# pghysels/STRUMPACK

Hardware: AMD Instinct MI355X
Metric: hss_compress_ulv_factor_solve_gflops (higher is better)
Workload: dtype f64

## Files before the change

### include/hssk.h

```cpp
#ifndef HSSK_H
#define HSSK_H

#ifdef __cplusplus
extern "C" {
#endif

typedef struct hssk_ctx hssk_ctx;

int hssk_ctx_create(hssk_ctx** ctx, int device);
void hssk_ctx_destroy(hssk_ctx* ctx);
void* hssk_ctx_stream(hssk_ctx* ctx);
int hssk_sync(hssk_ctx* ctx);
const char* hssk_last_error(void);
typedef struct hssk_plan hssk_plan;
int hssk_plan_begin(hssk_ctx* ctx, hssk_plan** plan);
int hssk_plan_end(hssk_ctx* ctx);
int hssk_plan_replay(hssk_ctx* ctx, hssk_plan* plan);
void hssk_plan_destroy(hssk_plan* plan);
int hssk_plan_size(const hssk_plan* plan);

void* hssk_malloc(long long bytes);
void hssk_free(void* dptr);
long long hssk_device_total_bytes(void);
int hssk_memcpy_h2d(hssk_ctx* ctx, void* dst, const void* src, long long bytes);
int hssk_memcpy_d2h(hssk_ctx* ctx, void* dst, const void* src, long long bytes);
int hssk_upload_async(hssk_ctx* ctx, void* dst, const void* src, long long bytes);
int hssk_memcpy_d2d(hssk_ctx* ctx, void* dst, const void* src, long long bytes);
int hssk_memcpy2d_h2d(hssk_ctx* ctx, void* dst, long long dpitch, const void* src, long long spitch,
                      long long width, long long height);
int hssk_memcpy2d_d2h(hssk_ctx* ctx, void* dst, long long dpitch, const void* src, long long spitch,
                      long long width, long long height);
int hssk_memset_zero(hssk_ctx* ctx, void* dst, long long bytes);
int hssk_h2d_block_async(hssk_ctx* ctx, double* dst, long long ldd, const double* src, long long lds, long long rows,
                         long long cols);
int hssk_h2d_bytes_async(hssk_ctx* ctx, void* dst, long long dpitch, const void* src, long long spitch, long long width,
                         long long cols);
int hssk_copy_fence(hssk_ctx* ctx);
int hssk_compute_fence(hssk_ctx* ctx);
int hssk_compute_mark(hssk_ctx* ctx, int slot);
int hssk_copy_wait(hssk_ctx* ctx, int slot);
int hssk_is_device_pointer(const void* ptr);
typedef struct hssk_aca_desc {
  const double* A;
  int lda, m, n;
  double rtol, atol;
  int max_rank, row0;
  double* U;
  int ldu;
  double* V;
  int ldv;
  int* rank;
} hssk_aca_desc;
int hssk_aca_vbatched(hssk_ctx* ctx, const hssk_aca_desc* descs, int count);
int hssk_side_begin(hssk_ctx* ctx);
int hssk_side_end(hssk_ctx* ctx);
int hssk_side_join(hssk_ctx* ctx);
int hssk_stream_wait(hssk_ctx* waiter, hssk_ctx* on);
int hssk_watch_start(hssk_ctx* ctx, int id);
int hssk_watch_stop(hssk_ctx* ctx, int id);
double hssk_watch_read_ms(hssk_ctx* ctx, int id, int* pairs);
float hssk_last_dgemm_ms(hssk_ctx* ctx);
double hssk_last_dgemm_flops(hssk_ctx* ctx);
int hssk_dgemm_timing_defer(hssk_ctx* ctx);
int hssk_dgemm_timing_collect(hssk_ctx* ctx, double* ms, double* flops, int* launches);
long long hssk_last_dgemm_trace(hssk_ctx* ctx, long long* out, long long max_wgs);
double hssk_last_dgemm_clock_ghz(hssk_ctx* ctx);

int hssk_fill_toeplitz(hssk_ctx* ctx, double* A, int n, long long lda, char kind);
int hssk_fill_toeplitz_block(hssk_ctx* ctx, double* A, int rows, int cols, long long lda, int i0, int j0, char kind);
int hssk_randn(hssk_ctx* ctx, double* P, int rows, long long cols, long long ld, int row0,
               long long stride, unsigned long long seed);

int hssk_dgemm(hssk_ctx* ctx, int transB, int m, long long n, long long k, double alpha,
               const double* A, long long lda, const double* B, long long ldb, double beta,
               double* C, long long ldc);

int hssk_sgemm_sketch(hssk_ctx* ctx, int transB, int m, long long n, long long k, double alpha,
                      const double* A, long long lda,
                      const float* B, long long ldb,
                      double beta, double* C, long long ldc);
int hssk_narrow_f32(hssk_ctx* ctx, float* dst, long long ldd, const double* src, long long lds, long long rows, long long cols);

#define HSSK_GEN_TOEPLITZ 1
#define HSSK_GEN_TOEPLITZ_UPPER 2
typedef struct hssk_gen {
  int kind, reserved;
  double p[4];
} hssk_gen;
int hssk_sketch_gen(hssk_ctx* ctx, const hssk_gen* g, int transG, int m, long long n, long long k, long long j0, double alpha,
                    const double* A, long long lda, double beta, double* C, long long ldc);
int hssk_gen_fill(hssk_ctx* ctx, const hssk_gen* g, double* A, long long rows, long long cols, long long lda, long long i0,
                  long long j0, int trans);

typedef struct hssk_gemm_desc {
  const double* A;
  const double* B;
  double* C;
  int m, n, k;
  int lda, ldb, ldc;
  int transA, transB;
  double alpha, beta;
} hssk_gemm_desc;
int hssk_gemm_vbatched(hssk_ctx* ctx, const hssk_gemm_desc* descs, int count);

typedef struct hssk_leaf_update_desc {
  const double* R;
  const double* D;
  double* Sr;
  double* Sc;
  int d, m, ldr, ldd, lds;
} hssk_leaf_update_desc;
int hssk_leaf_update_vbatched(hssk_ctx* ctx, const hssk_leaf_update_desc* descs, int count);

typedef struct hssk_kernel_spec {
  const double* X;
  long long n;
  int d, type, p;
  double h, lambda;
} hssk_kernel_spec;
typedef struct hssk_keval_desc {
  const int* ri;
  const int* ci;
  double* out;
  int nr, nc, ldo, r0, c0;
} hssk_keval_desc;
int hssk_kernel_eval_vbatched(hssk_ctx* ctx, const hssk_kernel_spec* spec, const hssk_keval_desc* descs, int count);
int hssk_knn(hssk_ctx* ctx, const double* X, int d, int n, int k, int q0, int q1, int* out_idx);
typedef struct hssk_colset_desc {
  const int* src0;
  const int* src1;
  int n0, n1, lo, hi;
  int* out;
  int* count;
  const int* n0_dev;
  const int* n1_dev;
} hssk_colset_desc;
int hssk_colsets(hssk_ctx* ctx, const hssk_colset_desc* descs, int count, int universe);
long long hssk_colsets_max_universe(void);
int hssk_cluster_median(hssk_ctx* ctx, double* X, int d, int n, int algo, int cluster_size, int* perm, int* status);
int hssk_kernel_predict(hssk_ctx* ctx, const hssk_kernel_spec* spec, const double* w, const double* T, int m, double* pred);
#define HSSK_KPREDICT_TAU 1.220703125e-4
int hssk_kernel_predict_f32(hssk_ctx* ctx, const float* X, long long n, int d, int type, int p, double h,
                            const float* w, const float* T, int m, float* pred, long long* stats);
int hssk_kernel_predict_splits(long long n, int m);

typedef struct hssk_colgather_desc {
  const double* src;
  double* dst;
  const int* idx;
  int rows, ncols, lds, ldd;
  int scatter;
} hssk_colgather_desc;
int hssk_gather_cols(hssk_ctx* ctx, const hssk_colgather_desc* descs, int count);
enum { HSSK_DT_F64 = 0, HSSK_DT_F32 = 1, HSSK_DT_C32 = 2, HSSK_DT_C64 = 3 };
int hssk_expand_image(hssk_ctx* ctx, double* dst, long long ldd, const void* src, long long lds, long long rows, long long cols,
                      int dtype);
typedef struct hssk_rowgather_desc {
  const double* src;
  double* dst;
  const int* idx;
  int nrows, cols, lds, ldd;
  int scatter, accumulate;
} hssk_rowgather_desc;
int hssk_gather_rows(hssk_ctx* ctx, const hssk_rowgather_desc* descs, int count);
typedef struct hssk_elem_desc {
  const double* A;
  long long lda;
  const int* I;
  const int* J;
  int i0, j0;
  double* B;
  int m, n, ldb, transpose;
  int rlo, rhi, clo, chi;
} hssk_elem_desc;
int hssk_gather_elems(hssk_ctx* ctx, const hssk_elem_desc* descs, int count);
int hssk_gather_elems_f32(hssk_ctx* ctx, const hssk_elem_desc* descs, int count);
int hssk_gen_elems(hssk_ctx* ctx, const hssk_gen* g, const hssk_elem_desc* descs, int count);
int hssk_sum_slabs(hssk_ctx* ctx, const double* slabs, long long count, long long stride, int nslab, double* out);
typedef struct hssk_transpose_desc {
  const double* src;
  double* dst;
  int rows, cols, lds, ldd;
} hssk_transpose_desc;
int hssk_transpose(hssk_ctx* ctx, const hssk_transpose_desc* descs, int count);

typedef struct hssk_triu_desc {
  const double* src;
  double* dst;
  int rows, cols, lds, ldd;
  int dstride;
} hssk_triu_desc;
int hssk_copy_triu(hssk_ctx* ctx, const hssk_triu_desc* descs, int count);

int hssk_sjlt_dense(hssk_ctx* ctx, double* Rt, int dn, long long K, long long ld, const int* pat, int nnz);
int hssk_sjlt_sketch(hssk_ctx* ctx, int transA, long long n_out, long long K, const double* A, long long lda,
                     const int* pat, int nnz, int dn, double* St, long long lds);

typedef struct hssk_combine_desc {
  const double *G0, *G1;
  int ldg, gsplit;
  const int* gidx;
  const double *M0, *M1;
  int ldm, msplit;
  const int* midx;
  const double* C;
  int csj, csk;
  double alpha;
  double* out;
  int ldo, rows, J, K;
} hssk_combine_desc;
int hssk_gather_combine(hssk_ctx* ctx, const hssk_combine_desc* descs, int count);

typedef struct hssk_ulvsplit_desc {
  const double* D;
  int ldd, m, r;
  const int* perm;
  const double* X;
  int ldx;
  double* W1;
  int ldw;
  double* W0t;
  int ldt;
} hssk_ulvsplit_desc;
int hssk_ulv_split(hssk_ctx* ctx, const hssk_ulvsplit_desc* descs, int count);
typedef struct hssk_ulvnode_desc {
  const double *B01, *B10, *Vt1a, *Vt1b, *Vd;
  double *Dh, *Vh;
  int ra, rb, rva, rvb;
  int eliminate;
  const int* perm;
  const double* X;
  double *W1, *Rlq, *Qt, *tau, *Vt0T, *Vt1, *Dt, *WQ;
  int m, r, rv, ldt;
} hssk_ulvnode_desc;
int hssk_ulv_node_vbatched(hssk_ctx* ctx, const hssk_ulvnode_desc* descs, int count);
int hssk_ulv_node_fits(int m, int r, int rv, int ra, int rb, int rva, int rvb);
long long hssk_ulv_node_launches(void);

typedef struct hssk_id_desc {
  double* W;
  int ldw, d, m;
  double rtol, atol;
  int max_rank;
  int* perm;
  int* rank;
  double* work;
  const double* src;
  int lds;
  int defer_x;
} hssk_id_desc;
int hssk_id_vbatched(hssk_ctx* ctx, const hssk_id_desc* descs, int count);
long long hssk_id_group_launches(void);
int hssk_id_solves_inline(int dmax, int mmax);
typedef struct hssk_xsolve_desc {
  const double* W;
  int ldw, rank, m;
  double* X;
  int ldx, solved;
} hssk_xsolve_desc;
int hssk_id_xsolve_vbatched(hssk_ctx* ctx, const hssk_xsolve_desc* descs, int count);
typedef struct hssk_pchol_desc {
  const double* G;
  int ldg, m;
  double rtol, atol;
  int max_rank;
  int* perm;
  int* rank;
  double* R;
  int ldr;
} hssk_pchol_desc;
int hssk_pchol_id_vbatched(hssk_ctx* ctx, const hssk_pchol_desc* descs, int count);
int hssk_pchol_id_max_m(void);
int hssk_pchol_id_rank_cap(int m);
typedef struct hssk_sum_desc {
  const double* P;
  long long stride, n;
  int count;
  double* out;
} hssk_sum_desc;
int hssk_sum_partials(hssk_ctx* ctx, const hssk_sum_desc* descs, int count);
typedef struct hssk_gram_desc {
  const double* W;
  int ldw, rows, m;
  double* G;
  int ldg;
} hssk_gram_desc;
int hssk_gram_vbatched(hssk_ctx* ctx, const hssk_gram_desc* descs, int count);
typedef struct hssk_gramgen_desc {
  const int* ri;
  int r0;
  const int* ci;
  int c0;
  int rows, m;
  double* G;
  int ldg;
} hssk_gramgen_desc;
int hssk_gram_gen_vbatched(hssk_ctx* ctx, const hssk_kernel_spec* spec, const hssk_gramgen_desc* descs, int count);
int hssk_gram_gen_supported(const hssk_kernel_spec* spec, int mmax);

typedef struct hssk_tnode {
  int c0, c1, lvl, reserved;
  double* S[2];
  int* perm[2];
  double* Rred[2];
  int* I[2];
  double* X[2];
  double *B01, *B10;
  double* W[2];
  int r[2], m[2], flag[2];
  int status, pad;
} hssk_tnode;
typedef struct hssk_elem_src {
  const double* A;
  long long lda;
  hssk_gen gen;
  int use_gen;
} hssk_elem_src;
int hssk_tree_inner(hssk_ctx* ctx, hssk_tnode* nodes, const int* order, int count, int d, int lds, int rcap, double rtol,
                    double atol, int max_rank, const hssk_elem_src* src, int* res);
int hssk_tree_rcap_max(void);

typedef struct hssk_qr_desc {
  double* A;
  int lda, rows, cols;
  double* Q;
  int ldq, nq;
  double* rdiag;
  double* work;
  int stair;
  double stop_rel, stop_abs;
  int r_only;
} hssk_qr_desc;
int hssk_qr_vbatched(hssk_ctx* ctx, const hssk_qr_desc* descs, int count);
typedef struct hssk_tpqr_desc {
  double* R1;
  int ld1;
  const double* R2;
  int ld2, m;
} hssk_tpqr_desc;
int hssk_tpqr_vbatched(hssk_ctx* ctx, const hssk_tpqr_desc* descs, int count);
int hssk_formq_vbatched(hssk_ctx* ctx, const hssk_qr_desc* descs, int count);

typedef struct hssk_trsm_desc {
  const double* T;
  double* B;
  int n, nrhs, ldt, ldb;
  int lower, transT, unit;
  const double* Tinv;
} hssk_trsm_desc;
int hssk_trsm_vbatched(hssk_ctx* ctx, const hssk_trsm_desc* descs, int count);
typedef struct hssk_lu_desc {
  double* A;
  int n, lda;
  int* piv;
  int* info;
} hssk_lu_desc;
int hssk_getrf_vbatched(hssk_ctx* ctx, const hssk_lu_desc* descs, int count);
typedef struct hssk_lusolve_desc {
  const double* LU;
  const int* piv;
  double* B;
  int n, nrhs, lda, ldb;
} hssk_lusolve_desc;
int hssk_getrs_vbatched(hssk_ctx* ctx, const hssk_lusolve_desc* descs, int count);
int hssk_laswp_vbatched(hssk_ctx* ctx, const hssk_lusolve_desc* descs, int count);

typedef struct hssk_blr_term {
  const double* U;
  const double* V;
  int r, n, src_off, src_flag;
} hssk_blr_term;
typedef struct hssk_blr_row {
  int first_term, nterms, off, m;
  const double* LU;
  int lda, mode;
  const int* piv;
  const double* Tinv;
} hssk_blr_row;
int hssk_blr_sweep(hssk_ctx* ctx, const hssk_blr_row* rows, int nrows, const hssk_blr_term* terms, int nterms, double* X, int* flags);
int hssk_blr_sweep_check(const hssk_blr_row* rows, int nrows, const hssk_blr_term* terms, int nterms);
int hssk_blr_sweep_resident(hssk_ctx* ctx, const hssk_blr_row* d_rows, int nrows, const hssk_blr_term* d_terms, double* X, int* flags);

int hssk_sweep_arm(hssk_ctx* ctx, double* handoff, long long count);
typedef struct hssk_sweep_fwd_desc {
  const double* fsrc;
  const double *B01, *B10, *zc;
  const int* permU;
  const double* XU;
  const double* Rlq;
  const double* Tinv;
  const double* WQ;
  const double* Vt0T;
  const int* permV;
  const double* XV;
  double *ft1, *y, *z;
  const double *LU, *TinvL, *TinvU;
  const int* piv;
  double* xroot;
  int ldf, rU0, rU1, rV0, rV1, ldz_in, m, r, mv, rv, ldp, ldz, ldxr;
  int wait0, wait1;
  const double* G;
  int ldg;
} hssk_sweep_fwd_desc;
int hssk_sweep_chain_ok(int m, int r, int mv, int rv);
long long hssk_sweep_chain_launches(void);
int hssk_ulv_fwd_sweep(hssk_ctx* ctx, const hssk_sweep_fwd_desc* descs, int count, int nrhs);
typedef struct hssk_sweep_bwd_desc {
  const double *Qt, *y, *xpart;
  double* out;
  int m, r, ldx, ldo;
  int wait0;
} hssk_sweep_bwd_desc;
int hssk_ulv_bwd_sweep(hssk_ctx* ctx, const hssk_sweep_bwd_desc* descs, int count, int nrhs);
typedef struct hssk_apply_up_desc {
  const double* src;
  const int* perm;
  const double* X;
  double* dst;
  int m, r, lds, ldd;
  int inner;
  int wait0, wait1;
} hssk_apply_up_desc;
typedef struct hssk_apply_down_desc {
  const double* tmp2;
  const int* perm;
  const double* X;
  const double *D, *x;
  const double *B01, *B10, *t1;
  double* out;
  double beta;
  int ld2, mo, ro, m, ldx, trans, ri_a, ri_b, ro_a, ro_b, ldt1, ldo;
  int wait0, wait1, wait2;
  int acc;
} hssk_apply_down_desc;
int hssk_apply_sweep(hssk_ctx* ctx, const hssk_apply_up_desc* ups, int nup, const hssk_apply_down_desc* downs, int ndown,
                     int nrhs);
int hssk_sweep_status(hssk_ctx* ctx);
int hssk_sweep_require_mma(hssk_ctx* ctx, int on);
int hssk_sweep_mma_min_nrhs(void);
long long hssk_sweep_mma_launches(void);
long long hssk_sweep_fused_launches(void);
long long hssk_sweep_fallbacks(void);
typedef struct hssk_trtri_desc {
  const double* R;
  double* Tinv;
  int n, ldr;
  int mode;
} hssk_trtri_desc;
int hssk_trtri_diag_vbatched(hssk_ctx* ctx, const hssk_trtri_desc* descs, int count);

typedef struct hssk_tree_node {
  int lo, m, c0, c1;
  int rU, rV, mU, mV;
  const double *XU, *XV;
  const int *ipermU, *ipermV;
  const double *B01, *B10, *D;
} hssk_tree_node;
typedef struct hssk_extract_block {
  int ri0, ni, cj0, nj;
  double* out;
  int ldo;
} hssk_extract_block;
int hssk_hss_extract(hssk_ctx* ctx, const hssk_tree_node* nodes, int root, int rmax, int maxdepth, const int* rows, int nrows,
                     const int* cols, int ncols, const hssk_extract_block* blocks, const long long* pair_off, int nblocks,
                     long long npairs, int accumulate, double* work);

typedef struct hssk_norm_desc {
  const double* P;
  int rows, cols, ld;
  double* out;
} hssk_norm_desc;
int hssk_sumsq_vbatched(hssk_ctx* ctx, const hssk_norm_desc* descs, int count);
typedef struct hssk_basis_desc {
  const double* X;
  const int* perm;
  double* out;
  int m, r, ldx, ldo;
} hssk_basis_desc;
int hssk_basis_dense(hssk_ctx* ctx, const hssk_basis_desc* descs, int count);
typedef struct hssk_shift_desc {
  double* A;
  int n, lda;
} hssk_shift_desc;
int hssk_shift_diag(hssk_ctx* ctx, const hssk_shift_desc* descs, int count, double sigma);
int hssk_shift_diag_cplx(hssk_ctx* ctx, const hssk_shift_desc* descs, int count, double re, double im);
double hssk_mfma_f64_peak_tflops(hssk_ctx* ctx, int iters);
int hssk_mfma_f64_probe(hssk_ctx* ctx, int iters, int waves_per_simd, int zero_data, double* out);

#ifdef __cplusplus
}
#endif
#endif
```

### strumpack_amd/csrc/host/hss_sources.cpp

```cpp
#include "hss_engine_internal.hpp"

namespace strumpack {
namespace HSS {

double DeviceHSS::Source::sketch_flops(const DeviceHSS& H, int dn) const {
  return 2.0 * products(H) * (double)H.n_ * (double)H.n_ * (H.sj_pat_ ? H.sj_nnz_ : dn);
}

struct DeviceHSS::DenseDeviceSource : DeviceHSS::Source {
  const double* dA;
  long long lda;
  DenseDeviceSource(const double* a, long long l) : dA(a), lda(l) {}
  bool extract_before_sample() const override { return true; }
  bool device_elems(const DeviceHSS&, hssk_elem_src* e) const override { e->A = dA; e->lda = lda; e->use_gen = 0; return true; }
  int done_products_ = 2;
  bool done_sparse_ = false;
  int products(const DeviceHSS&) const override { return done_products_; }
  double sketch_flops(const DeviceHSS& H, int dn) const override {
    return 2.0 * done_products_ * (double)H.n_ * (double)H.n_ * (done_sparse_ ? H.sj_nnz_ : dn);
  }
  void sample(DeviceHSS& H, int r0, int dn) override {
    const long long N = H.n_;
    long long j0 = 0, j1 = N;
    if (H.dist_subtree_) {
      const Node& c = H.nodes_[H.cut_nodes_[H.o_.rank]];
      j0 = c.lo; j1 = c.lo + c.m;
    } else if (H.o_.world > 1) {
      j0 = std::min(N, H.cols_per_rank_ * H.o_.rank); j1 = std::min(N, j0 + H.cols_per_rank_);
    }
    const long long nloc = j1 - j0;
    static const bool sj_dense = std::getenv("STRUMPACK_AMD_SJLT_DENSE") && std::atoi(std::getenv("STRUMPACK_AMD_SJLT_DENSE"));
    done_sparse_ = H.sj_pat_ && dn <= 1024 && !sj_dense;
    done_products_ = (!done_sparse_ && H.o_.symmetric) ? 1 : 2;
    if (nloc > 0 && done_sparse_) {
      for (int t = 0; t < 2; t++) {
        const double* Aop = t == 0 ? dA + j0 : dA + j0 * lda;
        double* St = (t == 0 ? H.Srt_ : H.Sct_) + r0 + j0 * H.dcap_;
        ck(hssk_sjlt_sketch(H.ctx_, t, nloc, N, Aop, lda, H.sj_pat_, H.sj_nnz_, dn, St, H.dcap_));
        ck(hssk_sync(H.ctx_));
        float ms = hssk_last_dgemm_ms(H.ctx_);
        if (ms > 0) {
          H.stats_.sketch_kernel_ms += ms; H.stats_.sketch_launches++;
          H.stats_.sketch_kernel_flops += hssk_last_dgemm_flops(H.ctx_);
          H.stats_.sketch_kernel_bytes += 8.0 * (double)nloc * (double)N;
        }
      }
    } else if (nloc > 0) {
      ck(hssk_dgemm(H.ctx_, 1, dn, nloc, N, 1.0, H.Rt_ + r0, H.dcap_, dA + j0, lda, 0.0, H.Srt_ + r0 + j0 * H.dcap_, H.dcap_));
      ck(hssk_dgemm_timing_defer(H.ctx_));
      if (H.o_.symmetric) {
        hssk_colgather_desc cp{H.Srt_ + r0 + j0 * H.dcap_, H.Sct_ + r0 + j0 * H.dcap_, nullptr, dn, (int)nloc, H.dcap_, H.dcap_, 0};
        ck(hssk_gather_cols(H.ctx_, &cp, 1));
      } else {
        ck(hssk_dgemm(H.ctx_, 0, dn, nloc, N, 1.0, H.Rt_ + r0, H.dcap_, dA + j0 * lda, lda, 0.0, H.Sct_ + r0 + j0 * H.dcap_, H.dcap_));
        ck(hssk_dgemm_timing_defer(H.ctx_));
      }
    }
    if (H.o_.world > 1 && !H.dist_subtree_) {
      const long long bytes = (long long)sizeof(double) * H.dcap_ * H.cols_per_rank_;
      H.comm(H.Srt_, bytes);
      H.comm(H.Sct_, bytes);
    }
  }
  void extract(DeviceHSS& H, const std::vector<ElemReq>& reqs) override {
    std::vector<hssk_elem_desc> d;
    d.reserve(reqs.size());
    for (auto& r : reqs)
      if (r.m > 0 && r.n > 0) d.push_back(hssk_elem_desc{dA, lda, r.dI, r.dJ, r.i0, r.j0, r.dB, r.m, r.n, r.ldb, 0});
    if (!d.empty()) ck(hssk_gather_elems(H.ctx_, d.data(), (int)d.size()));
  }
};

struct DeviceHSS::DenseDeviceSourceF32 : DeviceHSS::Source {
  const float* dA;
  long long lda;
  int route;
  double* dBuf = nullptr;
  long long nb = 0;
  int gen = -1;
  int done_products_ = 2;
  DenseDeviceSourceF32(const float* a, long long l, int r) : dA(a), lda(l), route(r) {}
  bool extract_before_sample() const override { return true; }
  bool device_elems(const DeviceHSS&, hssk_elem_src* e) const override {
    e->A = reinterpret_cast<const double*>(dA); e->lda = lda; e->use_gen = 2;
    return true;
  }
  int products(const DeviceHSS&) const override { return done_products_; }
  double sketch_flops(const DeviceHSS& H, int dn) const override { return 2.0 * done_products_ * (double)H.n_ * (double)H.n_ * dn; }
  void sample(DeviceHSS& H, int r0, int dn) override {
    if (H.o_.world > 1) throw std::invalid_argument("single-precision device operand: single-GPU only (multi-GPU float operands are not supported)");
    if (H.sj_pat_) throw std::invalid_argument("single-precision device operand: the SJLT sketch is not supported; use the Gaussian sketch");
    const long long N = H.n_;
    if (N <= 0 || dn <= 0) return;
    auto timed = [&](double bytes) {
      ck(hssk_dgemm_timing_defer(H.ctx_));
      H.stats_.sketch_kernel_bytes += bytes;
    };
    if (route == 1) {
      done_products_ = H.o_.symmetric ? 1 : 2;
      ck(hssk_sgemm_sketch(H.ctx_, 1, dn, N, N, 1.0, H.Rt_ + r0, H.dcap_, dA, lda, 0.0, H.Srt_ + r0, H.dcap_));
      timed(4.0 * (double)N * (double)N);
      if (H.o_.symmetric) {
        hssk_colgather_desc cp{H.Srt_ + r0, H.Sct_ + r0, nullptr, dn, (int)N, H.dcap_, H.dcap_, 0};
        ck(hssk_gather_cols(H.ctx_, &cp, 1));
      } else {
        ck(hssk_sgemm_sketch(H.ctx_, 0, dn, N, N, 1.0, H.Rt_ + r0, H.dcap_, dA, lda, 0.0, H.Sct_ + r0, H.dcap_));
        timed(4.0 * (double)N * (double)N);
      }
      return;
    }
    done_products_ = 2;
    if (gen != H.attempt_) {
      gen = H.attempt_;
      nb = std::max<long long>(64, (1LL << 30) / (8 * N) / 64 * 64);
      nb = std::min(nb, (N + 63) / 64 * 64);
      dBuf = H.work_->dbl((size_t)N * nb);
    }
    for (long long c0 = 0, b = 0; c0 < N; c0 += nb, b++) {
      const long long c1 = std::min(N, c0 + nb);
      ck(hssk_expand_image(H.ctx_, dBuf, N, dA + c0 * lda, lda, N, c1 - c0, HSSK_DT_F32));
      ck(hssk_dgemm(H.ctx_, 0, dn, c1 - c0, N, 1.0, H.Rt_ + r0, H.dcap_, dBuf, N, 0.0, H.Sct_ + r0 + c0 * H.dcap_, H.dcap_));
      timed(0.);
      ck(hssk_dgemm(H.ctx_, 1, dn, N, c1 - c0, 1.0, H.Rt_ + r0 + c0 * H.dcap_, H.dcap_, dBuf, N, b ? 1.0 : 0.0, H.Srt_ + r0, H.dcap_));
      timed(0.);
    }
  }
  void extract(DeviceHSS& H, const std::vector<ElemReq>& reqs) override {
    std::vector<hssk_elem_desc> d;
    d.reserve(reqs.size());
    for (auto& r : reqs)
      if (r.m > 0 && r.n > 0) d.push_back(hssk_elem_desc{reinterpret_cast<const double*>(dA), lda, r.dI, r.dJ, r.i0, r.j0, r.dB, r.m, r.n, r.ldb, 0});
    if (!d.empty()) ck(hssk_gather_elems_f32(H.ctx_, d.data(), (int)d.size()));
  }
};

struct DeviceHSS::ShardedDenseSource : DeviceHSS::Source {
  const double* dRows;
  long long ldr;
  const double* dCols;
  long long ldc;
  ShardedDenseSource(const double* r, long long lr, const double* c, long long lc) : dRows(r), ldr(lr), dCols(c), ldc(lc) {}
  bool device_elems(const DeviceHSS& H, hssk_elem_src* e) const override {
    const Node& c = H.nodes_[H.o_.world == 1 ? 0 : H.cut_nodes_[H.o_.rank]];
    e->A = dCols - (long long)c.lo * ldc; e->lda = ldc; e->use_gen = 0;
    return true;
  }
  void sample(DeviceHSS& H, int r0, int dn) override {
    const bool single = H.o_.world == 1;
    if (!single && !H.dist_subtree_) throw std::invalid_argument("sharded operand: the tree cannot be cut into one subtree per rank (world must be a power of two and the tree complete down to that depth)");
    if (H.sj_pat_) throw std::invalid_argument("sharded operand: the SJLT sketch needs the replicated-operand interface");
    const long long N = H.n_;
    const Node& c = H.nodes_[single ? 0 : H.cut_nodes_[H.o_.rank]];
    const long long j0 = c.lo, nloc = c.m;
    auto timed = [&] { ck(hssk_dgemm_timing_defer(H.ctx_)); };
    ck(hssk_dgemm(H.ctx_, 0, dn, nloc, N, 1.0, H.Rt_ + r0, H.dcap_, dCols, ldc, 0.0, H.Sct_ + r0 + j0 * H.dcap_, H.dcap_));
    timed();
    if (dRows) {
      ck(hssk_dgemm(H.ctx_, 1, dn, nloc, N, 1.0, H.Rt_ + r0, H.dcap_, dRows, ldr, 0.0, H.Srt_ + r0 + j0 * H.dcap_, H.dcap_));
      timed();
    } else {
      H.tmp_->rewind();
      double* P = H.tmp_->dbl((size_t)dn * N);
      double* mineP = H.tmp_->dbl((size_t)dn * nloc);
      ck(hssk_dgemm(H.ctx_, 1, dn, N, nloc, 1.0, H.Rt_ + r0 + j0 * H.dcap_, H.dcap_, dCols, ldc, 0.0, P, dn));
      timed();
      const double tc = now();
      std::vector<long long> offs(H.o_.world), counts(H.o_.world);
      for (int g = 0; g < H.o_.world; g++) {
        const Node& cg = H.nodes_[single ? 0 : H.cut_nodes_[g]];
        offs[g] = (long long)cg.lo * dn; counts[g] = (long long)cg.m * dn;
      }
      H.reduce_scatter_sum(P, offs, counts, mineP);
      hssk_colgather_desc cp{mineP, H.Srt_ + r0 + j0 * H.dcap_, nullptr, dn, (int)nloc, dn, H.dcap_, 0};
      ck(hssk_gather_cols(H.ctx_, &cp, 1));
      ck(hssk_sync(H.ctx_));
      H.stats_.t_comm += now() - tc;
    }
  }
  void extract(DeviceHSS& H, const std::vector<ElemReq>& reqs) override {
    const Node& c = H.nodes_[H.o_.world == 1 ? 0 : H.cut_nodes_[H.o_.rank]];
    const int j0 = c.lo, j1 = c.lo + c.m;
    auto inside = [&](const std::vector<int>* h, int i0, int cnt) {
      if (!h) return i0 >= j0 && i0 + cnt <= j1;
      for (int i = 0; i < cnt; i++) if ((*h)[i] < j0 || (*h)[i] >= j1) return false;
      return true;
    };
    std::vector<hssk_elem_desc> own, part, back;
    size_t tot = 0;
    for (auto& r : reqs) if (r.m > 0 && r.n > 0 && !(inside(r.hI, r.i0, r.m) && inside(r.hJ, r.j0, r.n))) tot += (size_t)r.m * r.n;
    double* stage = tot ? H.comm_arena_->dbl(tot) : nullptr;
    size_t off = 0;
    for (auto& r : reqs) {
      if (r.m <= 0 || r.n <= 0) continue;
      if (inside(r.hI, r.i0, r.m) && inside(r.hJ, r.j0, r.n)) {
        own.push_back(hssk_elem_desc{dCols - (long long)j0 * ldc, ldc, r.dI, r.dJ, r.i0, r.j0, r.dB, r.m, r.n, r.ldb, 0, 0, 0, 0, 0});
      } else {
        double* T = stage + off;
        off += (size_t)r.m * r.n;
        if (dRows) part.push_back(hssk_elem_desc{dRows - j0, ldr, r.dI, r.dJ, r.i0, r.j0, T, r.m, r.n, r.m, 0, j0, j1, 0, 0});
        else part.push_back(hssk_elem_desc{dCols - (long long)j0 * ldc, ldc, r.dI, r.dJ, r.i0, r.j0, T, r.m, r.n, r.m, 0, 0, 0, j0, j1});
        back.push_back(hssk_elem_desc{T, r.m, nullptr, nullptr, 0, 0, r.dB, r.m, r.n, r.ldb, 0, 0, 0, 0, 0});
      }
    }
    if (!own.empty()) ck(hssk_gather_elems(H.ctx_, own.data(), (int)own.size()));
    if (!part.empty()) {
      const double tc = now();
      ck(hssk_gather_elems(H.ctx_, part.data(), (int)part.size()));
      H.allreduce_sum(stage, (long long)tot);
      ck(hssk_gather_elems(H.ctx_, back.data(), (int)back.size()));
      H.stats_.t_comm += now() - tc;
    }
  }
};

struct DeviceHSS::HostBlockSource : DeviceHSS::Source {
  const void* hA;
  long long lda;
  int dtype = HSSK_DT_F64;
  const host_fill_t* fill;
  const host_elem_t* elem;
  double* dBuf[2] = {nullptr, nullptr};
  double* dNat[2] = {nullptr, nullptr};
  long long nb = 0;
  int gen = -1;
  std::vector<double*> dcache;
  HostBlockSource(const void* a, long long l, const host_fill_t* f, const host_elem_t* e, int dt = HSSK_DT_F64)
      : hA(a), lda(l), dtype(dt), fill(f), elem(e) {}
  long long reals() const { return dtype == HSSK_DT_C32 || dtype == HSSK_DT_C64 ? 2 : 1; }
  size_t esize() const { return dtype == HSSK_DT_F32 ? 4 : dtype == HSSK_DT_C64 ? 16 : 8; }
  double image_at(size_t I, size_t J) const {
    switch (dtype) {
      case HSSK_DT_F32: return (double)((const float*)hA)[I + J * (size_t)lda];
      case HSSK_DT_C32: {
        const float* z = (const float*)hA + 2 * (I / 2 + (J / 2) * (size_t)lda);
        return (I & 1) == (J & 1) ? (double)z[0] : ((I & 1) ? (double)z[1] : -(double)z[1]);
      }
      case HSSK_DT_C64: {
        const double* z = (const double*)hA + 2 * (I / 2 + (J / 2) * (size_t)lda);
        return (I & 1) == (J & 1) ? z[0] : ((I & 1) ? z[1] : -z[1]);
      }
      default: return ((const double*)hA)[I + J * (size_t)lda];
    }
  }
  void sample(DeviceHSS& H, int r0, int dn) override {
    if (H.o_.world > 1) throw std::invalid_argument("host-resident operands are single-GPU (use the device / sharded interfaces)");
    const long long N = H.n_;
    const bool typed = hA && dtype != HSSK_DT_F64;
    const long long W = typed ? reals() : 1, ns = N / W;
    if (typed && N % W) throw std::logic_error("image dimension of a complex operand must be even");
    const bool first = gen != H.attempt_;
    if (first) {
      gen = H.attempt_;
      long long bytes = 1536LL << 20;
      if (const char* e = std::getenv("STRUMPACK_AMD_HOST_BLOCK_MB")) bytes = std::max(1LL, std::atoll(e)) << 20;
      if (const char* e = std::getenv("STRUMPACK_AMD_HOST_BLOCK_KB")) bytes = std::max(1LL, std::atoll(e)) << 10;
      nb = std::max<long long>(64, bytes / (8 * std::max<long long>(N, 1)) / 64 * 64);
      nb = std::min(nb, (N + 63) / 64 * 64);
      dBuf[0] = H.work_->dbl((size_t)N * nb);
      if (!typed) dBuf[1] = H.work_->dbl((size_t)N * nb);
      else for (int k = 0; k < 2; k++) dNat[k] = H.work_->dbl(((size_t)ns * (size_t)(nb / W) * esize() + 7) / 8);
    }
    const long long nblk = (N + nb - 1) / nb;
    const bool capture = first;
    if (capture) {
      dcache.assign(H.nodes_.size(), nullptr);
      for (size_t id = 0; id < H.nodes_.size(); id++)
        if (H.nodes_[id].leaf() && H.nodes_[id].m > 0) dcache[id] = H.work_->dbl((size_t)H.nodes_[id].m * H.nodes_[id].m);
    }
    std::vector<double> tmp;
    auto upload = [&](long long b) {
      const long long c0 = b * nb, c1 = std::min(N, c0 + nb);
      if (typed)
        ck(hssk_h2d_bytes_async(H.ctx_, dNat[b & 1], (long long)(ns * esize()), (const char*)hA + (size_t)(c0 / W) * lda * esize(),
                                (long long)(lda * esize()), (long long)(ns * esize()), (c1 - c0) / W));
      else if (hA) ck(hssk_h2d_block_async(H.ctx_, dBuf[b & 1], N, (const double*)hA + (size_t)c0 * lda, lda, N, c1 - c0));
      else {
        tmp.resize((size_t)N * (c1 - c0));
        (*fill)(c0, c1, tmp.data());
        ck(hssk_h2d_block_async(H.ctx_, dBuf[b & 1], N, tmp.data(), N, N, c1 - c0));
      }
    };
    upload(0);
    for (long long b = 0; b < nblk; b++) {
      const long long c0 = b * nb, c1 = std::min(N, c0 + nb);
      ck(hssk_copy_fence(H.ctx_));
      const double* Ab = typed ? dBuf[0] : dBuf[b & 1];
      if (typed) {
        ck(hssk_expand_image(H.ctx_, dBuf[0], N, dNat[b & 1], ns, ns, (c1 - c0) / W, dtype));
        ck(hssk_compute_mark(H.ctx_, (int)(b & 1)));
      }
      ck(hssk_dgemm(H.ctx_, 0, dn, c1 - c0, N, 1.0, H.Rt_ + r0, H.dcap_, Ab, N, 0.0, H.Sct_ + r0 + c0 * H.dcap_, H.dcap_));
      ck(hssk_dgemm(H.ctx_, 1, dn, N, c1 - c0, 1.0, H.Rt_ + r0 + c0 * H.dcap_, H.dcap_, Ab, N, b ? 1.0 : 0.0, H.Srt_ + r0, H.dcap_));
      if (capture) {
        std::vector<hssk_colgather_desc> dg;
        for (size_t id = 0; id < H.nodes_.size(); id++) {
          const Node& nd = H.nodes_[id];
          if (!dcache[id]) continue;
          const long long a = std::max<long long>(nd.lo, c0), e = std::min<long long>(nd.lo + nd.m, c1);
          if (a >= e) continue;
          dg.push_back(hssk_colgather_desc{Ab + nd.lo + (size_t)(a - c0) * N, dcache[id] + (size_t)(a - nd.lo) * nd.m, nullptr, nd.m, (int)(e - a),
                                           (int)N, nd.m, 0});
        }
        if (!dg.empty()) ck(hssk_gather_cols(H.ctx_, dg.data(), (int)dg.size()));
      }
      if (!typed) ck(hssk_compute_mark(H.ctx_, (int)(b & 1)));
      if (b + 1 < nblk) {
        ck(hssk_copy_wait(H.ctx_, (int)((b + 1) & 1)));
        upload(b + 1);
      }
    }
    ck(hssk_sync(H.ctx_));
  }
  void extract(DeviceHSS& H, const std::vector<ElemReq>& reqs) override {
    std::vector<size_t> off(reqs.size() + 1, 0);
    for (size_t k = 0; k < reqs.size(); k++) off[k + 1] = off[k] + (size_t)std::max(reqs[k].m, 0) * std::max(reqs[k].n, 0);
    std::vector<const double*> hit(reqs.size(), nullptr);
    if (!dcache.empty()) {
      std::vector<std::pair<int, size_t>> by_lo;
      for (size_t id = 0; id < H.nodes_.size(); id++) if (dcache[id]) by_lo.push_back({H.nodes_[id].lo, id});
      std::sort(by_lo.begin(), by_lo.end());
      std::vector<hssk_colgather_desc> cp;
      for (size_t k = 0; k < reqs.size(); k++) {
        const ElemReq& r = reqs[k];
        if (r.hI || r.hJ || r.i0 != r.j0 || r.m != r.n || r.m <= 0 || gen != H.attempt_) continue;
        auto it = std::lower_bound(by_lo.begin(), by_lo.end(), std::make_pair(r.i0, size_t(0)));
        if (it == by_lo.end() || it->first != r.i0 || H.nodes_[it->second].m != r.m) continue;
        hit[k] = dcache[it->second];
        cp.push_back(hssk_colgather_desc{hit[k], r.dB, nullptr, r.m, r.n, r.m, r.ldb, 0});
      }
      if (!cp.empty()) ck(hssk_gather_cols(H.ctx_, cp.data(), (int)cp.size()));
    }
    for (size_t k = 0; k < reqs.size(); k++)
      if (hit[k]) off[k + 1] = off[k];
      else off[k + 1] = off[k] + (size_t)std::max(reqs[k].m, 0) * std::max(reqs[k].n, 0);
    std::unique_ptr<double[]> img_store(new double[std::max<size_t>(off.back(), 1)]);
    struct { double* p; double* data() { return p; } } img{img_store.get()};
    host_parallel_for(reqs.size(), [&](size_t k) {
      const ElemReq& r = reqs[k];
      if (r.m <= 0 || r.n <= 0 || hit[k]) return;
      double* B = img.data() + off[k];
      if (hA && dtype != HSSK_DT_F64) {
        for (int j = 0; j < r.n; j++) {
          const size_t J = (size_t)(r.hJ ? (*r.hJ)[j] : r.j0 + j);
          for (int i = 0; i < r.m; i++) B[i + (size_t)j * r.m] = image_at((size_t)(r.hI ? (*r.hI)[i] : r.i0 + i), J);
        }
      } else if (hA) {
        for (int j = 0; j < r.n; j++) {
          const double* col = (const double*)hA + (size_t)(r.hJ ? (*r.hJ)[j] : r.j0 + j) * lda;
          if (r.hI) for (int i = 0; i < r.m; i++) B[i + (size_t)j * r.m] = col[(*r.hI)[i]];
          else std::memcpy(B + (size_t)j * r.m, col + r.i0, sizeof(double) * r.m);
        }
      } else {
        std::vector<int> I(r.m), J(r.n);
        for (int i = 0; i < r.m; i++) I[i] = r.hI ? (*r.hI)[i] : r.i0 + i;
        for (int j = 0; j < r.n; j++) J[j] = r.hJ ? (*r.hJ)[j] : r.j0 + j;
        (*elem)(r.m, I.data(), r.n, J.data(), B, r.m);
      }
    });
    for (size_t k = 0; k < reqs.size(); k++) {
      const ElemReq& r = reqs[k];
      if (r.m <= 0 || r.n <= 0 || hit[k]) continue;
      if (r.ldb == r.m) ck(hssk_upload_async(H.ctx_, r.dB, img.data() + off[k], (long long)(sizeof(double) * (off[k + 1] - off[k]))));
      else ck(hssk_memcpy2d_h2d(H.ctx_, r.dB, sizeof(double) * r.ldb, img.data() + off[k], sizeof(double) * r.m, sizeof(double) * r.m, r.n));
    }
  }
};

struct DeviceHSS::CallbackSource : DeviceHSS::Source {
  const host_mult_t* mult;
  const host_sample_t* usample = nullptr;
  const host_elem_t& elem;
  CallbackSource(const host_mult_t& m, const host_elem_t& e) : mult(&m), elem(e) {}
  CallbackSource(const host_sample_t& s, const host_elem_t& e) : mult(nullptr), usample(&s), elem(e) {}
  void sample(DeviceHSS& H, int r0, int dn) override {
    if (H.o_.world > 1) throw std::invalid_argument("the host-callback interface is single-GPU");
    if (usample) {
      const int N = H.n_;
      if (N == 0 || dn == 0) return;
      std::vector<double> R((size_t)N * dn), Sr((size_t)N * dn), Sc((size_t)N * dn);
      (*usample)(N, dn, R.data(), Sr.data(), Sc.data());
      double* dT = H.tmp_->dbl((size_t)N * dn);
      const double* src[3] = {R.data(), Sr.data(), Sc.data()};
      double* dst[3] = {H.Rt_ + r0, H.Srt_ + r0, H.Sct_ + r0};
      for (int q = 0; q < 3; q++) {
        ck(hssk_memcpy_h2d(H.ctx_, dT, src[q], (long long)(sizeof(double) * (size_t)N * dn)));
        hssk_transpose_desc b{dT, dst[q], N, dn, N, H.dcap_};
        ck(hssk_transpose(H.ctx_, &b, 1));
        ck(hssk_sync(H.ctx_));
      }
      return;
    }
    const int N = H.n_;
    if (N == 0 || dn == 0) return;
    double* dT = H.tmp_->dbl((size_t)N * dn);
    std::vector<double> R((size_t)N * dn), S((size_t)N * dn);
    hssk_transpose_desc t{H.Rt_ + r0, dT, dn, N, H.dcap_, N};
    ck(hssk_transpose(H.ctx_, &t, 1));
    ck(hssk_memcpy_d2h(H.ctx_, R.data(), dT, (long long)(sizeof(double) * R.size())));
    for (int pass = 0; pass < 2; pass++) {
      (*mult)(pass == 0 ? 'N' : 'C', N, dn, R.data(), N, S.data(), N);
      ck(hssk_memcpy_h2d(H.ctx_, dT, S.data(), (long long)(sizeof(double) * S.size())));
      hssk_transpose_desc b{dT, (pass == 0 ? H.Srt_ : H.Sct_) + r0, N, dn, N, H.dcap_};
      ck(hssk_transpose(H.ctx_, &b, 1));
      ck(hssk_sync(H.ctx_));
    }
  }
  void extract(DeviceHSS& H, const std::vector<ElemReq>& reqs) override {
    for (auto& r : reqs) {
      if (r.m <= 0 || r.n <= 0) continue;
      std::vector<int> I(r.m), J(r.n);
      for (int i = 0; i < r.m; i++) I[i] = r.hI ? (*r.hI)[i] : r.i0 + i;
      for (int j = 0; j < r.n; j++) J[j] = r.hJ ? (*r.hJ)[j] : r.j0 + j;
      std::vector<double> B((size_t)r.m * r.n);
      elem(r.m, I.data(), r.n, J.data(), B.data(), r.m);
      ck(hssk_memcpy2d_h2d(H.ctx_, r.dB, sizeof(double) * r.ldb, B.data(), sizeof(double) * r.m, sizeof(double) * r.m, r.n));
    }
  }
};

struct DeviceHSS::GeneratorSource : DeviceHSS::Source {
  hssk_gen g;
  explicit GeneratorSource(const hssk_gen& g_) : g(g_) {}
  bool extract_before_sample() const override { return true; }
  bool device_elems(const DeviceHSS&, hssk_elem_src* e) const override { e->A = nullptr; e->lda = 0; e->gen = g; e->use_gen = 1; return true; }
  int products(const DeviceHSS& H) const override { return H.o_.symmetric ? 1 : 2; }
  void sample(DeviceHSS& H, int r0, int dn) override {
    if (H.sj_pat_) throw std::invalid_argument("generated operand: the SJLT sketch streams a stored matrix; use the Gaussian sketch");
    const long long N = H.n_;
    long long j0 = 0, j1 = N;
    if (H.dist_subtree_) {
      const Node& c = H.nodes_[H.cut_nodes_[H.o_.rank]];
      j0 = c.lo; j1 = c.lo + c.m;
    } else if (H.o_.world > 1) {
      j0 = std::min(N, H.cols_per_rank_ * H.o_.rank); j1 = std::min(N, j0 + H.cols_per_rank_);
    }
    const long long nloc = j1 - j0;
    auto timed = [&] { ck(hssk_dgemm_timing_defer(H.ctx_)); };
    if (nloc > 0) {
      ck(hssk_sketch_gen(H.ctx_, &g, 1, dn, nloc, N, j0, 1.0, H.Rt_ + r0, H.dcap_, 0.0, H.Srt_ + r0 + j0 * H.dcap_, H.dcap_));
      timed();
      if (H.o_.symmetric) {
        hssk_colgather_desc cp{H.Srt_ + r0 + j0 * H.dcap_, H.Sct_ + r0 + j0 * H.dcap_, nullptr, dn, (int)nloc, H.dcap_, H.dcap_, 0};
        ck(hssk_gather_cols(H.ctx_, &cp, 1));
      } else {
        ck(hssk_sketch_gen(H.ctx_, &g, 0, dn, nloc, N, j0, 1.0, H.Rt_ + r0, H.dcap_, 0.0, H.Sct_ + r0 + j0 * H.dcap_, H.dcap_));
        timed();
      }
    }
    if (H.o_.world > 1 && !H.dist_subtree_) {
      const long long bytes = (long long)sizeof(double) * H.dcap_ * H.cols_per_rank_;
      H.comm(H.Srt_, bytes);
      H.comm(H.Sct_, bytes);
    }
  }
  void extract(DeviceHSS& H, const std::vector<ElemReq>& reqs) override {
    std::vector<hssk_elem_desc> d;
    d.reserve(reqs.size());
    for (auto& r : reqs)
      if (r.m > 0 && r.n > 0) d.push_back(hssk_elem_desc{nullptr, 0, r.dI, r.dJ, r.i0, r.j0, r.dB, r.m, r.n, r.ldb, 0});
    if (!d.empty()) ck(hssk_gen_elems(H.ctx_, &g, d.data(), (int)d.size()));
  }
};

void DeviceHSS::compress_generator(const hssk_gen& g) {
  GeneratorSource s(g);
  check_symmetry(s);
  compress(s);
}
void DeviceHSS::check_symmetry(Source& src) {
  if (o_.symmetric != 2 || n_ < 2) return;
  const int q = std::min(512, n_);
  std::vector<int> I(q), J(q);
  std::minstd_rand g(12345);
  for (int i = 0; i < q; i++) { I[i] = (int)(g() % (unsigned)n_); J[i] = (int)(g() % (unsigned)n_); }
  tmp_->rewind();
  int* dI = tmp_->ints(q);
  int* dJ = tmp_->ints(q);
  double* B1 = tmp_->dbl((size_t)q * q);
  double* B2 = tmp_->dbl((size_t)q * q);
  ck(hssk_memcpy_h2d(ctx_, dI, I.data(), (long long)sizeof(int) * q));
  ck(hssk_memcpy_h2d(ctx_, dJ, J.data(), (long long)sizeof(int) * q));
  std::vector<ElemReq> rq{ElemReq{dI, dJ, &I, &J, 0, 0, q, q, B1, q}, ElemReq{dJ, dI, &J, &I, 0, 0, q, q, B2, q}};
  src.extract(*this, rq);
  std::vector<double> h1((size_t)q * q), h2((size_t)q * q);
  ck(hssk_memcpy_d2h(ctx_, h1.data(), B1, (long long)sizeof(double) * q * q));
  ck(hssk_memcpy_d2h(ctx_, h2.data(), B2, (long long)sizeof(double) * q * q));
  double dmax = 0, amax = 0;
  for (int j = 0; j < q; j++)
    for (int i = 0; i < q; i++) {
      dmax = std::max(dmax, std::abs(h1[i + (size_t)j * q] - h2[j + (size_t)i * q]));
      amax = std::max(amax, std::abs(h1[i + (size_t)j * q]));
    }
  if (dmax > 1e-14 * std::max(amax, 1e-300)) throw std::invalid_argument("compress: the operand was declared symmetric and is not (sampled entries differ from their mirror images)");
}

void DeviceHSS::compress_dense_device(const double* dA, long long lda) {
  DenseDeviceSource s(dA, lda);
  check_symmetry(s);
  compress(s);
}
void DeviceHSS::compress_dense_device_f32(const float* dA, long long lda, int precision) {
  if (precision < 0 || precision > 2) throw std::invalid_argument("compress_dense_device_f32: sketch precision must be 0 (auto), 1 (FP32 matrix cores) or 2 (exact)");
  if (o_.world > 1) throw std::invalid_argument("compress_dense_device_f32: single-GPU only (multi-GPU float operands are not supported)");
  if (o_.sketch == 1) throw std::invalid_argument("compress_dense_device_f32: the SJLT sketch is not supported on a float operand; use the Gaussian sketch");
  if (!dA || lda < n_) throw std::invalid_argument("compress_dense_device_f32: bad operand");
  const int route = precision ? precision : (o_.rel_tol >= ((double)n_ + 4.) * std::ldexp(1., -24) ? 1 : 2);
  f32_route_ = route;
  DenseDeviceSourceF32 s(dA, lda, route);
  check_symmetry(s);
  compress(s);
}
void DeviceHSS::compress_dense_host(const double* A, long long lda) {
  HostBlockSource s(A, lda, nullptr, nullptr);
  compress(s);
}
void DeviceHSS::compress_dense_host_typed(const void* A, long long lda, int dtype) {
  if (dtype != HSSK_DT_F32 && dtype != HSSK_DT_C32 && dtype != HSSK_DT_C64) throw std::invalid_argument("compress_dense_host_typed: unknown scalar type");
  HostBlockSource s(A, lda, nullptr, nullptr, dtype);
  compress(s);
}
void DeviceHSS::compress_host_blocks(const host_fill_t& fill, const host_elem_t& elem) {
  HostBlockSource s(nullptr, 0, &fill, &elem);
  compress(s);
}
void DeviceHSS::compress_dense_device_sharded(const double* dRows, long long ldr, const double* dCols, long long ldc) {
  if (!dCols) throw std::invalid_argument("sharded operand: the column block is required");
  ShardedDenseSource s(dRows, ldr, dCols, ldc);
  compress(s);
}
bool DeviceHSS::shard_range(int rank, int& lo, int& hi) const {
  if (o_.world == 1) { lo = 0; hi = n_; return true; }
  if (!dist_subtree_ || rank < 0 || rank >= (int)cut_nodes_.size()) return false;
  lo = nodes_[cut_nodes_[rank]].lo;
  hi = lo + nodes_[cut_nodes_[rank]].m;
  return true;
}
void DeviceHSS::compress_callbacks_user_random(const host_sample_t& sample, const host_elem_t& elem) {
  if (!o_.user_random) throw std::logic_error("compress_callbacks_user_random: the engine was not built with user_random");
  CallbackSource s(sample, elem);
  compress(s);
}
void DeviceHSS::compress_callbacks(const host_mult_t& mult, const host_elem_t& elem) {
  CallbackSource s(mult, elem);
  compress(s);
}

}
}
```

### strumpack_amd/csrc/kernels/hssk_ctx.hip

```cpp
#include "hssk_internal.h"

#include <cstdlib>
#include <unistd.h>

#include <atomic>
#include <condition_variable>
#include <functional>
#include <mutex>
#include <thread>
#include <vector>

static thread_local std::string g_err;
static std::mutex g_pool_mu;
static std::vector<hssk_ctx*> g_pool;
void hssk_set_error(const std::string& msg) { g_err = msg; }

thread_local std::vector<std::function<void()>>* hssk_rec::sink = nullptr;

struct hssk_uploader {
  static constexpr int SLOTS = 4;
  static constexpr size_t CHUNK = size_t(256) << 20;
  hssk_rt::stream_t copy{};
  hssk_rt::event_t ev_copy{}, ev_compute{};
  hssk_rt::event_t ev_mark[2];
  bool marked[2] = {false, false};
  char* pinned[SLOTS] = {nullptr, nullptr, nullptr, nullptr};
  hssk_rt::event_t slot_ev[SLOTS];
  bool slot_busy[SLOTS] = {false, false, false, false};
  int next = 0;
  hssk_uploader() {
    copy = hssk_rt::stream_create();
    ev_copy = hssk_rt::event_create();
    ev_compute = hssk_rt::event_create();
    ev_mark[0] = hssk_rt::event_create();
    ev_mark[1] = hssk_rt::event_create();
    for (int i = 0; i < SLOTS; i++) slot_ev[i] = hssk_rt::event_create();
  }
  char* slot(int s) {
    if (!pinned[s]) pinned[s] = (char*)hssk_rt::pinned_malloc(CHUNK);
    return pinned[s];
  }
  void release_slots() {
    try { hssk_rt::sync(copy); } catch (...) {}
    for (int i = 0; i < SLOTS; i++) {
      if (pinned[i]) hssk_rt::pinned_free(pinned[i]);
      pinned[i] = nullptr;
      slot_busy[i] = false;
    }
  }
  ~hssk_uploader() {
    try { hssk_rt::sync(copy); } catch (...) {}
    for (int i = 0; i < SLOTS; i++) { if (pinned[i]) hssk_rt::pinned_free(pinned[i]); hssk_rt::event_destroy(slot_ev[i]); }
    hssk_rt::event_destroy(ev_copy);
    hssk_rt::event_destroy(ev_compute);
    hssk_rt::event_destroy(ev_mark[0]);
    hssk_rt::event_destroy(ev_mark[1]);
    hssk_rt::stream_destroy(copy);
  }
};
static hssk_uploader* uploader(hssk_ctx* c) {
  if (!c->uploader) c->uploader = new hssk_uploader();
  return c->uploader;
}
class PackPool {
 public:
  explicit PackPool(unsigned n) : n_(n), pid_(getpid()) {
    for (unsigned t = 0; t < n_; t++) th_.emplace_back([this, t] { loop(t); });
  }
  ~PackPool() {
    if (getpid() != pid_) { for (auto& t : th_) t.detach(); return; }
    { std::lock_guard<std::mutex> g(mu_); stop_ = true; gen_++; }
    cv_.notify_all();
    for (auto& t : th_) t.join();
  }
  unsigned size() const { return n_; }
  void run(const std::function<void(unsigned)>& fn) {
    if (getpid() != pid_) { for (unsigned t = 0; t < n_; t++) fn(t); return; }
    std::lock_guard<std::mutex> own(owner_);
    std::unique_lock<std::mutex> lk(mu_);
    fn_ = &fn; pending_ = n_; gen_++;
    cv_.notify_all();
    done_.wait(lk, [&] { return pending_ == 0; });
  }

 private:
  void loop(unsigned t) {
    unsigned long seen = 0;
    for (;;) {
      const std::function<void(unsigned)>* f;
      {
        std::unique_lock<std::mutex> lk(mu_);
        cv_.wait(lk, [&] { return gen_ != seen; });
        seen = gen_;
        if (stop_) return;
        f = fn_;
      }
      (*f)(t);
      { std::lock_guard<std::mutex> g(mu_); if (--pending_ == 0) done_.notify_all(); }
    }
  }
  unsigned n_;
  const pid_t pid_;
  std::vector<std::thread> th_;
  std::mutex mu_, owner_;
  std::condition_variable cv_, done_;
  const std::function<void(unsigned)>* fn_ = nullptr;
  unsigned long gen_ = 0;
  unsigned pending_ = 0;
  bool stop_ = false;
};
static PackPool& pack_pool() {
  static PackPool p(std::max(1u, std::min(24u, std::thread::hardware_concurrency())));
  return p;
}
static void host_pack(char* dst, const char* src, size_t spitch, size_t colb, long long c0, long long c1) {
  const long long ncol = c1 - c0;
  const size_t total = colb * (size_t)ncol;
  if (total < (size_t(8) << 20)) {
    for (long long j = 0; j < ncol; j++) std::memcpy(dst + colb * j, src + (size_t)(c0 + j) * spitch, colb);
    return;
  }
  PackPool& pool = pack_pool();
  const unsigned nt = pool.size();
  const size_t per = (total + nt - 1) / nt;
  pool.run([=](unsigned t) {
    size_t b0 = std::min(total, per * t), b1 = std::min(total, b0 + per);
    while (b0 < b1) {
      const size_t j = b0 / colb, o = b0 % colb, len = std::min(colb - o, b1 - b0);
      std::memcpy(dst + b0, src + (size_t)(c0 + (long long)j) * spitch + o, len);
      b0 += len;
    }
  });
}
static void h2d_bytes(hssk_ctx* c, char* dst, size_t dpitch, const char* src, size_t spitch, size_t colb, long long cols) {
  hssk_uploader* u = uploader(c);
  if (hssk_rt::is_pinned_host_pointer(src)) {
    if (dpitch == colb && spitch == colb) hssk_rt::h2d(dst, src, colb * (size_t)cols, u->copy);
    else hssk_rt::h2d_2d(dst, dpitch, src, spitch, colb, (size_t)cols, u->copy);
    return;
  }
  static const bool direct = [] { const char* e = std::getenv("HSSK_H2D_DIRECT"); return !(e && e[0] == '0'); }();
  if (direct && dpitch == colb && spitch == colb) {
    hssk_rt::h2d(dst, src, colb * (size_t)cols, u->copy);
    return;
  }
  if (colb > hssk_uploader::CHUNK) {
    for (long long j = 0; j < cols; j++)
      for (size_t o = 0; o < colb; o += hssk_uploader::CHUNK) {
        const size_t len = std::min(hssk_uploader::CHUNK, colb - o);
        const int s = u->next; u->next = (s + 1) % hssk_uploader::SLOTS;
        if (u->slot_busy[s]) hssk_rt::event_sync(u->slot_ev[s]);
        std::memcpy(u->slot(s), src + (size_t)j * spitch + o, len);
        hssk_rt::h2d(dst + (size_t)j * dpitch + o, u->slot(s), len, u->copy);
        hssk_rt::event_record(u->slot_ev[s], u->copy);
        u->slot_busy[s] = true;
      }
    return;
  }
  const long long cpc = std::max<long long>(1, (long long)(hssk_uploader::CHUNK / colb));
  for (long long c0 = 0; c0 < cols; c0 += cpc) {
    const long long c1 = std::min(cols, c0 + cpc);
    const int s = u->next; u->next = (s + 1) % hssk_uploader::SLOTS;
    if (u->slot_busy[s]) hssk_rt::event_sync(u->slot_ev[s]);
    host_pack(u->slot(s), src, spitch, colb, c0, c1);
    if (dpitch == colb)
      hssk_rt::h2d(dst + (size_t)c0 * dpitch, u->slot(s), colb * (size_t)(c1 - c0), u->copy);
    else
      hssk_rt::h2d_2d(dst + (size_t)c0 * dpitch, dpitch, u->slot(s), colb, colb, (size_t)(c1 - c0), u->copy);
    hssk_rt::event_record(u->slot_ev[s], u->copy);
    u->slot_busy[s] = true;
  }
}

extern "C" {

int hssk_h2d_block_async(hssk_ctx* c, double* dst, long long ldd, const double* src, long long lds, long long rows,
                         long long cols) {
  HSSK_API_BEGIN
  if (rows <= 0 || cols <= 0) return 0;
  h2d_bytes(c, (char*)dst, sizeof(double) * (size_t)ldd, (const char*)src, sizeof(double) * (size_t)lds, sizeof(double) * (size_t)rows, cols);
  HSSK_API_END
}
int hssk_h2d_bytes_async(hssk_ctx* c, void* dst, long long dpitch, const void* src, long long spitch, long long width, long long cols) {
  HSSK_API_BEGIN
  if (width <= 0 || cols <= 0) return 0;
  if (dpitch < width || spitch < width) HSSK_UNSUPPORTED("pitch smaller than the row width");
  h2d_bytes(c, (char*)dst, (size_t)dpitch, (const char*)src, (size_t)spitch, (size_t)width, cols);
  HSSK_API_END
}
int hssk_copy_fence(hssk_ctx* c) {
  HSSK_API_BEGIN
  hssk_uploader* u = uploader(c);
  hssk_rt::event_record(u->ev_copy, u->copy);
  hssk_rt::stream_wait_event(c->stream, u->ev_copy);
  HSSK_API_END
}
int hssk_compute_fence(hssk_ctx* c) {
  HSSK_API_BEGIN
  hssk_uploader* u = uploader(c);
  hssk_rt::event_record(u->ev_compute, c->stream);
  hssk_rt::stream_wait_event(u->copy, u->ev_compute);
  HSSK_API_END
}
int hssk_compute_mark(hssk_ctx* c, int slot) {
  HSSK_API_BEGIN
  hssk_uploader* u = uploader(c);
  hssk_rt::event_record(u->ev_mark[slot & 1], c->stream);
  u->marked[slot & 1] = true;
  HSSK_API_END
}
int hssk_copy_wait(hssk_ctx* c, int slot) {
  HSSK_API_BEGIN
  hssk_uploader* u = uploader(c);
  if (u->marked[slot & 1]) hssk_rt::stream_wait_event(u->copy, u->ev_mark[slot & 1]);
  HSSK_API_END
}

const char* hssk_last_error(void) { return g_err.c_str(); }

int hssk_ctx_create(hssk_ctx** out, int device) {
  HSSK_API_BEGIN
  if (hssk_rt::device_count() <= device)
    throw std::runtime_error("hssk_ctx_create: no HIP device " + std::to_string(device) +
                             " (this library has no CPU fallback)");
  hssk_rt::set_device(device);
  {
    std::lock_guard<std::mutex> g(g_pool_mu);
    for (size_t i = 0; i < g_pool.size(); i++)
      if (g_pool[i]->device == device) {
        *out = g_pool[i];
        g_pool.erase(g_pool.begin() + i);
        return 0;
      }
  }
  hssk_ctx* c = new hssk_ctx;
  c->device = device;
  c->stream = hssk_rt::stream_create();
  c->ring_bytes = size_t(64) << 20;
  c->h_ring = (char*)hssk_rt::pinned_malloc(c->ring_bytes);
  c->zero_copy_bytes = hssk_rt::pinned_is_device_visible() ? 65536 : 0;
  if (const char* e = std::getenv("HSSK_ZERO_COPY_BYTES")) c->zero_copy_bytes = (size_t)std::atoll(e);
  c->d_ring = (char*)hssk_rt::dev_malloc(c->ring_bytes);
  c->ev0 = hssk_rt::event_create();
  c->ev1 = hssk_rt::event_create();
  c->ev_sync = hssk_rt::event_create();
  *out = c;
  HSSK_API_END
}

void hssk_ctx_destroy(hssk_ctx* c) {
  if (!c) return;
  try { hssk_rt::sync(c->stream); } catch (...) {}
  {
    std::lock_guard<std::mutex> g(g_pool_mu);
    if (g_pool.size() < 8) {
      if (c->uploader) c->uploader->release_slots();
      c->ring_off = 0;
      c->dgemm_timed = false;
      if (c->on_side) { c->stream = c->main_saved; c->on_side = false; }
      for (int i = 0; i < 8; i++) {
        for (auto& p : c->watch[i]) { c->watch_free.push_back(p.first); c->watch_free.push_back(p.second); }
        c->watch[i].clear();
        c->watch_open[i] = false;
      }
      c->recording = nullptr;
      c->require_mma = false;
      g_pool.push_back(c);
      return;
    }
  }
  hssk_rt::pinned_free(c->h_ring);
  hssk_rt::dev_free(c->d_ring);
  hssk_rt::dev_free(c->d_scratch);
  hssk_rt::dev_free(c->d_aux);
  hssk_rt::dev_free(c->d_gen);
  delete c->uploader;
  hssk_rt::pinned_free(c->h_sweep_err);
  for (auto& w : c->watch) for (auto& p : w) { hssk_rt::event_destroy(p.first); hssk_rt::event_destroy(p.second); }
  for (auto& b : c->dgemm_deferred) { hssk_rt::event_destroy(b.a); hssk_rt::event_destroy(b.b); }
  for (auto e : c->watch_free) hssk_rt::event_destroy(e);
  hssk_rt::event_destroy(c->ev0);
  hssk_rt::event_destroy(c->ev_sync);
  if (c->side_made) { hssk_rt::event_destroy(c->ev_fork); hssk_rt::event_destroy(c->ev_join); hssk_rt::stream_destroy(c->side); }
  hssk_rt::event_destroy(c->ev1);
  hssk_rt::stream_destroy(c->stream);
  delete c;
}

void* hssk_ctx_stream(hssk_ctx* c) { return (void*)c->stream; }

int hssk_stream_wait(hssk_ctx* waiter, hssk_ctx* on) {
  HSSK_API_BEGIN
  if (!waiter || !on) throw std::invalid_argument("hssk_stream_wait: null context");
  if (waiter == on) return 0;
  hssk_rt::event_record(on->ev_sync, on->stream);
  hssk_rt::stream_wait_event(waiter->stream, on->ev_sync);
  HSSK_API_END
}
int hssk_side_begin(hssk_ctx* c) {
  HSSK_API_BEGIN
  if (c->on_side) throw std::logic_error("hssk_side_begin: already on the side stream");
  if (!c->side_made) {
    c->side = hssk_rt::stream_create();
    c->ev_fork = hssk_rt::event_create();
    c->ev_join = hssk_rt::event_create();
    c->side_made = true;
  }
  auto f = [c]() {
    hssk_rt::event_record(c->ev_fork, c->stream);
    hssk_rt::stream_wait_event(c->side, c->ev_fork);
    c->main_saved = c->stream;
    c->stream = c->side;
    c->on_side = true;
  };
  f();
  if (hssk_rec::sink) hssk_rec::sink->push_back(f);
  HSSK_API_END
}
int hssk_side_end(hssk_ctx* c) {
  HSSK_API_BEGIN
  if (!c->on_side) throw std::logic_error("hssk_side_end: not on the side stream");
  auto f = [c]() { c->stream = c->main_saved; c->on_side = false; };
  f();
  if (hssk_rec::sink) hssk_rec::sink->push_back(f);
  HSSK_API_END
}
int hssk_side_join(hssk_ctx* c) {
  HSSK_API_BEGIN
  if (c->on_side) throw std::logic_error("hssk_side_join: still on the side stream");
  if (!c->side_made) return 0;
  auto f = [c]() {
    hssk_rt::event_record(c->ev_join, c->side);
    hssk_rt::stream_wait_event(c->stream, c->ev_join);
  };
  f();
  if (hssk_rec::sink) hssk_rec::sink->push_back(f);
  HSSK_API_END
}
static hssk_rt::event_t watch_event(hssk_ctx* c) {
  if (c->watch_free.empty()) return hssk_rt::event_create();
  hssk_rt::event_t e = c->watch_free.back();
  c->watch_free.pop_back();
  return e;
}
int hssk_watch_start(hssk_ctx* c, int id) {
  HSSK_API_BEGIN
  if (id < 0 || id >= 8) throw std::invalid_argument("hssk_watch_start: id out of range");
  if (c->watch_open[id]) {
    auto p = c->watch[id].back();
    c->watch[id].pop_back();
    c->watch_free.push_back(p.first);
    c->watch_free.push_back(p.second);
    c->watch_open[id] = false;
  }
  hssk_rt::event_t a = watch_event(c), b = watch_event(c);
  hssk_rt::event_record(a, c->stream);
  c->watch[id].emplace_back(a, b);
  c->watch_open[id] = true;
  HSSK_API_END
}
int hssk_watch_stop(hssk_ctx* c, int id) {
  HSSK_API_BEGIN
  if (id < 0 || id >= 8 || !c->watch_open[id]) throw std::logic_error("hssk_watch_stop: stopwatch is not running");
  hssk_rt::event_record(c->watch[id].back().second, c->stream);
  c->watch_open[id] = false;
  HSSK_API_END
}
double hssk_watch_read_ms(hssk_ctx* c, int id, int* pairs) {
  if (pairs) *pairs = 0;
  if (!c || id < 0 || id >= 8) return 0.;
  try {
    if (c->watch_open[id]) { hssk_rt::event_record(c->watch[id].back().second, c->stream); c->watch_open[id] = false; }
    hssk_rt::sync(c->stream);
    double ms = 0.;
    for (auto& p : c->watch[id]) {
      ms += hssk_rt::event_elapsed_ms(p.first, p.second);
      c->watch_free.push_back(p.first);
      c->watch_free.push_back(p.second);
    }
    if (pairs) *pairs = (int)c->watch[id].size();
    c->watch[id].clear();
    return ms;
  } catch (const std::exception& e) { hssk_set_error(e.what()); return -1.; }
}

int hssk_sync(hssk_ctx* c) {
  HSSK_API_BEGIN
  hssk_rt::sync(c->stream);
  HSSK_API_END
}

void* hssk_malloc(long long bytes) {
  try { return hssk_rt::dev_malloc((size_t)bytes); } catch (const std::exception& e) { hssk_set_error(e.what()); return nullptr; }
}
void hssk_free(void* p) { hssk_rt::dev_free(p); }
long long hssk_device_total_bytes(void) {
  try { return (long long)hssk_rt::device_total_bytes(); } catch (...) { return 0; }
}

int hssk_memcpy_h2d(hssk_ctx* c, void* dst, const void* src, long long bytes) {
  HSSK_API_BEGIN
  hssk_rt::h2d(dst, src, (size_t)bytes, c->stream);
  hssk_rt::sync(c->stream);
  HSSK_API_END
}
int hssk_upload_async(hssk_ctx* c, void* dst, const void* src, long long bytes) {
  HSSK_API_BEGIN
  if (bytes <= 0) return 0;
  const size_t need = ((size_t)bytes + 255) & ~size_t(255);
  if (need > c->ring_bytes) {
    hssk_rt::h2d(dst, src, (size_t)bytes, c->stream);
    hssk_rt::sync(c->stream);
    return 0;
  }
  if (c->ring_off + need > c->ring_bytes) { hssk_rt::sync(c->stream); c->ring_off = 0; }
  std::memcpy(c->h_ring + c->ring_off, src, (size_t)bytes);
  hssk_rt::h2d(dst, c->h_ring + c->ring_off, (size_t)bytes, c->stream);
  c->ring_off += need;
  HSSK_API_END
}
int hssk_memcpy_d2h(hssk_ctx* c, void* dst, const void* src, long long bytes) {
  HSSK_API_BEGIN
  hssk_rt::d2h(dst, src, (size_t)bytes, c->stream);
  hssk_rt::sync(c->stream);
  HSSK_API_END
}

int hssk_memcpy_d2d(hssk_ctx* c, void* dst, const void* src, long long bytes) {
  HSSK_API_BEGIN
  hssk_rt::d2d(dst, src, (size_t)bytes, c->stream);
  HSSK_API_END
}
int hssk_memcpy2d_h2d(hssk_ctx* c, void* dst, long long dpitch, const void* src, long long spitch,
                      long long width, long long height) {
  HSSK_API_BEGIN
  hssk_rt::h2d_2d(dst, (size_t)dpitch, src, (size_t)spitch, (size_t)width, (size_t)height, c->stream);
  hssk_rt::sync(c->stream);
  HSSK_API_END
}
int hssk_memcpy2d_d2h(hssk_ctx* c, void* dst, long long dpitch, const void* src, long long spitch,
                      long long width, long long height) {
  HSSK_API_BEGIN
  hssk_rt::d2h_2d(dst, (size_t)dpitch, src, (size_t)spitch, (size_t)width, (size_t)height, c->stream);
  hssk_rt::sync(c->stream);
  HSSK_API_END
}
int hssk_memset_zero(hssk_ctx* c, void* dst, long long bytes) {
  HSSK_API_BEGIN
  hssk_rt::memset_async(dst, 0, (size_t)bytes, c->stream);
  HSSK_API_END
}
int hssk_is_device_pointer(const void* p) { return hssk_rt::is_device_pointer(p) ? 1 : 0; }

double hssk_last_dgemm_clock_ghz(hssk_ctx* c) {
  try {
    if (!c->d_clk) return 0.;
    long long h[2] = {0, 0};
    hssk_rt::d2h(h, c->d_clk, sizeof(h), c->stream);
    hssk_rt::sync(c->stream);
    return h[1] > 0 ? (double)h[0] / ((double)h[1] / 100e6) * 1e-9 : 0.;
  } catch (...) { return 0.; }
}

long long hssk_last_dgemm_trace(hssk_ctx* c, long long* out, long long max_wgs) {
  try {
    if (!c->d_clk || c->dgemm_trace_wgs <= 0) return 0;
    const long long nw = c->dgemm_trace_wgs < max_wgs ? c->dgemm_trace_wgs : max_wgs;
    if (nw > 0) { hssk_rt::d2h(out, c->d_clk + 4, sizeof(long long) * 4 * nw, c->stream); hssk_rt::sync(c->stream); }
    return nw;
  } catch (...) { return -1; }
}

int hssk_plan_begin(hssk_ctx* c, hssk_plan** out) {
  try {
    if (c->recording || hssk_rec::sink) throw std::logic_error("hssk_plan_begin: a plan is already being recorded");
    if (!hssk_rt::pinned_is_device_visible()) throw std::runtime_error("hssk_plan_begin: pinned memory is not device-visible here");
    hssk_plan* p = new hssk_plan();
    c->recording = p;
    hssk_rec::sink = &p->launches;
    *out = p;
    return 0;
  } catch (const std::exception& e) { hssk_set_error(e.what()); return 1; }
}
int hssk_plan_end(hssk_ctx* c) {
  c->recording = nullptr;
  hssk_rec::sink = nullptr;
  return 0;
}
int hssk_plan_replay(hssk_ctx* c, hssk_plan* p) {
  try {
    if (c->recording) throw std::logic_error("hssk_plan_replay: cannot replay while recording");
    for (auto& f : p->launches) f();
    hssk_rt::check_launch();
    return 0;
  } catch (const std::exception& e) { hssk_set_error(e.what()); return 1; }
}
void hssk_plan_destroy(hssk_plan* p) { delete p; }
int hssk_plan_size(const hssk_plan* p) { return p ? (int)p->launches.size() : 0; }

double hssk_last_dgemm_flops(hssk_ctx* c) { return c->dgemm_timed ? c->dgemm_timed_flops : 0.; }

float hssk_last_dgemm_ms(hssk_ctx* c) {
  if (!c->dgemm_timed) return -1.f;
  try { return hssk_rt::event_elapsed_ms(c->ev0, c->ev1); } catch (...) { return -1.f; }
}

int hssk_dgemm_timing_defer(hssk_ctx* c) {
  HSSK_API_BEGIN
  if (!c->dgemm_timed) return 0;
  c->dgemm_deferred.push_back(hssk_ctx::TimedBracket{c->ev0, c->ev1, c->dgemm_timed_flops});
  c->ev0 = watch_event(c);
  c->ev1 = watch_event(c);
  c->dgemm_timed = false;
  HSSK_API_END
}
int hssk_dgemm_timing_collect(hssk_ctx* c, double* ms, double* flops, int* launches) {
  HSSK_API_BEGIN
  double t = 0., f = 0.;
  int n = 0;
  if (!c->dgemm_deferred.empty()) hssk_rt::sync(c->stream);
  for (auto& b : c->dgemm_deferred) {
    const float e = hssk_rt::event_elapsed_ms(b.a, b.b);
    if (e > 0) { t += e; f += b.flops; n++; }
    c->watch_free.push_back(b.a);
    c->watch_free.push_back(b.b);
  }
  c->dgemm_deferred.clear();
  if (ms) *ms = t;
  if (flops) *flops = f;
  if (launches) *launches = n;
  HSSK_API_END
}

}
```

### strumpack_amd/csrc/kernels/hssk_dgemm.hip

```cpp
#include "hssk_device.h"
#include "hssk_internal.h"
#include "hssk_gen.h"

#include <algorithm>
#include <cstdlib>
#include <type_traits>

namespace {

constexpr int BN = 64, BK = 16;

template <int BM, bool TRANSB, bool FULL, int TAG = 0>
__global__ __launch_bounds__(256, 2) void dgemm_kernel(int m, long long n, long long k, const double* __restrict__ A,
                                                       long long lda, const double* __restrict__ B, long long ldb,
                                                       double* __restrict__ P, long long ldp, long long pstride,
                                                       long long kchunk, int jtile0, long long* __restrict__ clk) {
  const long long t0_ = clk ? hssk_clock() : 0, w0_ = clk ? hssk_wallclock() : 0;
  constexpr int LDA_S = BM + 16, LDB_S = BN + 16;
  constexpr int WM = BM / 2;
  constexpr int MT = WM / 16;
  constexpr int NT = 2;
  constexpr int A_PER_THREAD = BM * BK / 256;
  constexpr int B_PER_THREAD = BN * BK / 256;
  constexpr int A2 = A_PER_THREAD / 2, B2 = B_PER_THREAD / 2;
  HSSK_SHARED double As[2 * BK * LDA_S];
  HSSK_SHARED double Bs[2 * BK * LDB_S];

  const int tid = threadIdx.x, lane = tid & 63, wave = tid >> 6;
  const int l15 = lane & 15, l4 = lane >> 4;
  int bx = blockIdx.x;
  {
    const int nx = gridDim.x, x = bx & 7, q = nx >> 3, r = nx & 7;
    bx = x * q + (x < r ? x : r) + (bx >> 3);
  }
  const long long j0 = (long long)(bx + jtile0) * BN;
  const int i0 = blockIdx.y * BM;
  const long long kbeg = (long long)blockIdx.z * kchunk;
  const long long kend = kbeg + kchunk < k ? kbeg + kchunk : k;
  const int wm = (wave & 1) * WM, wn = (wave >> 1) * 32;

  hssk_d4 acc[MT][NT];
#pragma unroll
  for (int a = 0; a < MT; a++)
#pragma unroll
    for (int b = 0; b < NT; b++) acc[a][b] = hssk_d4{0., 0., 0., 0.};

  const double* Ak = A + i0 + kbeg * lda;
  const double* Bk = TRANSB ? B + j0 + kbeg * ldb : B + j0 * ldb + kbeg;
  const long long stepA = (long long)BK * lda, stepB = TRANSB ? (long long)BK * ldb : (long long)BK;
  const long long nst = (kend - kbeg + BK - 1) / BK;

  auto compute = [&](int buf) {
    const double* as = As + buf * BK * LDA_S + wm + l15;
    const double* bs = Bs + buf * BK * LDB_S + wn + l15;
    double af[2][MT], bf[2][NT];
#pragma unroll
    for (int a = 0; a < MT; a++) af[0][a] = as[l4 * LDA_S + a * 16];
#pragma unroll
    for (int b = 0; b < NT; b++) bf[0][b] = bs[l4 * LDB_S + b * 16];
#pragma unroll
    for (int ks = 0; ks < BK; ks += 4) {
      const int cur = (ks >> 2) & 1, nxt = cur ^ 1;
      if (ks + 4 < BK) {
#pragma unroll
        for (int a = 0; a < MT; a++) af[nxt][a] = as[(ks + 4 + l4) * LDA_S + a * 16];
#pragma unroll
        for (int b = 0; b < NT; b++) bf[nxt][b] = bs[(ks + 4 + l4) * LDB_S + b * 16];
      }
#pragma unroll
      for (int a = 0; a < MT; a++)
#pragma unroll
        for (int b = 0; b < NT; b++)
          acc[a][b] = hssk_mfma_f64_16x16x4(bf[cur][b], af[cur][a], acc[a][b]);
    }
  };

  if (FULL) {
    int offA[A2], ldsA[A2], offB[B2], ldsB[B2];
#pragma unroll
    for (int r = 0; r < A2; r++) {
      int e = tid + 256 * r;
      int i = 2 * (e % (BM / 2)), kk = e / (BM / 2);
      offA[r] = i + kk * (int)lda;
      ldsA[r] = kk * LDA_S + i;
    }
#pragma unroll
    for (int r = 0; r < B2; r++) {
      int e = tid + 256 * r;
      if (TRANSB) {
        int j = 2 * (e % (BN / 2)), kk = e / (BN / 2);
        offB[r] = j + kk * (int)ldb;
        ldsB[r] = kk * LDB_S + j;
      } else {
        int kk = 2 * (e % (BK / 2)), j = e / (BK / 2);
        offB[r] = kk + j * (int)ldb;
        ldsB[r] = kk * LDB_S + j;
      }
    }
    hssk_d2 ra0[A2], rb0[B2], ra1[A2], rb1[B2];
    auto load = [&](hssk_d2 (&ra)[A2], hssk_d2 (&rb)[B2]) {
#pragma unroll
      for (int r = 0; r < A2; r++) ra[r] = *reinterpret_cast<const hssk_d2*>(Ak + offA[r]);
#pragma unroll
      for (int r = 0; r < B2; r++) rb[r] = *reinterpret_cast<const hssk_d2*>(Bk + offB[r]);
      Ak += stepA; Bk += stepB;
    };
    auto store = [&](int buf, const hssk_d2 (&ra)[A2], const hssk_d2 (&rb)[B2]) {
      double* as = As + buf * BK * LDA_S;
      double* bs = Bs + buf * BK * LDB_S;
#pragma unroll
      for (int r = 0; r < A2; r++) *reinterpret_cast<hssk_d2*>(as + ldsA[r]) = ra[r];
#pragma unroll
      for (int r = 0; r < B2; r++) {
        if (TRANSB) *reinterpret_cast<hssk_d2*>(bs + ldsB[r]) = rb[r];
        else { bs[ldsB[r]] = rb[r][0]; bs[ldsB[r] + LDB_S] = rb[r][1]; }
      }
    };
    load(ra0, rb0);
    store(0, ra0, rb0);
    if (nst > 1) load(ra1, rb1);
    __syncthreads();
    long long st = 0;
    for (; st + 2 < nst; st += 2) {
      load(ra0, rb0);
      compute(0);
      store(1, ra1, rb1);
      __syncthreads();
      if (st + 3 < nst) load(ra1, rb1);
      compute(1);
      store(0, ra0, rb0);
      __syncthreads();
    }
    compute(0);
    if (st + 1 < nst) {
      store(1, ra1, rb1);
      __syncthreads();
      compute(1);
    }
  } else {
    double ra[A_PER_THREAD], rb[B_PER_THREAD];
    auto load = [&](long long k0) {
#pragma unroll
      for (int r = 0; r < A_PER_THREAD; r++) {
        int e = tid + 256 * r;
        int i = e % BM, kk = e / BM;
        ra[r] = (i0 + i < m && k0 + kk < kend) ? A[i0 + i + (k0 + kk) * lda] : 0.;
      }
#pragma unroll
      for (int r = 0; r < B_PER_THREAD; r++) {
        int e = tid + 256 * r;
        if (TRANSB) {
          int j = e % BN, kk = e / BN;
          rb[r] = (j0 + j < n && k0 + kk < kend) ? B[j0 + j + (k0 + kk) * ldb] : 0.;
        } else {
          int kk = e % BK, j = e / BK;
          rb[r] = (j0 + j < n && k0 + kk < kend) ? B[k0 + kk + (j0 + j) * ldb] : 0.;
        }
      }
    };
    auto store = [&](int buf) {
      double* as = As + buf * BK * LDA_S;
      double* bs = Bs + buf * BK * LDB_S;
#pragma unroll
      for (int r = 0; r < A_PER_THREAD; r++) {
        int e = tid + 256 * r;
        as[(e / BM) * LDA_S + (e % BM)] = ra[r];
      }
#pragma unroll
      for (int r = 0; r < B_PER_THREAD; r++) {
        int e = tid + 256 * r;
        if (TRANSB) bs[(e / BN) * LDB_S + (e % BN)] = rb[r];
        else bs[(e % BK) * LDB_S + (e / BK)] = rb[r];
      }
    };
    if (nst > 0) { load(kbeg); store(0); }
    __syncthreads();
    int buf = 0;
    long long k0 = kbeg;
    for (long long st = 0; st + 1 < nst; st++) {
      k0 += BK;
      load(k0);
      compute(buf);
      store(buf ^ 1);
      __syncthreads();
      buf ^= 1;
    }
    if (nst > 0) compute(buf);
  }
  double* Pz = P + (long long)blockIdx.z * pstride;
#pragma unroll
  for (int a = 0; a < MT; a++)
#pragma unroll
    for (int b = 0; b < NT; b++)
#pragma unroll
      for (int r = 0; r < 4; r++) {
        int gi = i0 + wm + a * 16 + l15;
        long long gj = j0 + wn + b * 16 + l4 + 4 * r;
        if (gi < m && gj < n) Pz[gi + gj * ldp] = acc[a][b][r];
      }
  if (clk && threadIdx.x == 0) {
    const long long w1 = hssk_wallclock();
    if (blockIdx.x == 0 && blockIdx.y == 0 && blockIdx.z == 0) {
      clk[0] = hssk_clock() - t0_;
      clk[1] = w1 - w0_;
    }
    const long long fid = blockIdx.x + (long long)gridDim.x * (blockIdx.y + (long long)gridDim.y * blockIdx.z);
    long long* rec = clk + 4 + 4 * fid;
    rec[0] = w0_; rec[1] = w1; rec[2] = hssk_hwid(); rec[3] = bx;
  }
}

template <int MBLK, bool TRANSB, int TAG = 0, bool GEN = false>
__global__ __launch_bounds__(512, 2) void sketch_kernel(long long n, long long k, const double* __restrict__ A, long long lda,
                                                        const double* __restrict__ B, long long ldb,
                                                        double* __restrict__ P, long long ldp, long long pstride,
                                                        long long kchunk, int jtile0, long long* __restrict__ clk,
                                                        hssk_gen gen, long long jg0) {
  const long long t0_ = clk ? hssk_clock() : 0, w0_ = clk ? hssk_wallclock() : 0;
  constexpr int BM = 64 * MBLK, BN2 = 128;
  constexpr int WM = BM / 2, MT = WM / 16, NT = 2;
  constexpr int A_DBL = BM * BK, B_DBL = BN2 * BK, SLOT = A_DBL + B_DBL;
  constexpr int NCH = GEN ? MBLK : MBLK + 2;
  constexpr bool KJ_IMAGE = TRANSB && !GEN;
  HSSK_DYN_SHARED(double, lds);

  const int tid = threadIdx.x, lane = tid & 63, wave = hssk_uniform(tid >> 6);
  const int l15 = lane & 15, l4 = lane >> 4;
  int bx = blockIdx.x;
  {
    const int nx = gridDim.x, x = bx & 7, q = nx >> 3, r = nx & 7;
    bx = x * q + (x < r ? x : r) + (bx >> 3);
  }
  const long long j0 = (long long)(bx + jtile0) * BN2;
  const int i0 = blockIdx.y * BM;
  const long long kbeg = (long long)blockIdx.z * kchunk;
  const long long kend = kbeg + kchunk < k ? kbeg + kchunk : k;
  const int nst = (int)((kend - kbeg) / BK);
  const int wm = (wave & 1) * WM, wn = (wave >> 1) * 32;

  const int kk = lane >> 5, pos = 2 * (lane & 31);
  const double* srcA = A + i0 + (pos ^ (16 * kk)) + (kbeg + 2 * wave + kk) * lda;
  const long long stepA = (long long)BK * lda;
  const double* srcB[2] = {nullptr, nullptr};
  long long stepB = 0;
  if (GEN) {
  } else if (TRANSB) {
    const long long jp = j0 + (pos ^ (16 * kk));
    srcB[0] = B + (jp < n - 2 ? jp : n - 2) + (kbeg + 2 * wave + kk) * ldb;
    srcB[1] = B + (jp + 64 < n - 2 ? jp + 64 : n - 2) + (kbeg + 2 * wave + kk) * ldb;
    stepB = (long long)BK * ldb;
  } else {
#pragma unroll
    for (int r = 0; r < 2; r++) {
      const int j = 8 * (wave + 8 * r) + (lane >> 3), q = lane & 7;
      const long long jc = j0 + j < n - 1 ? j0 + j : n - 1;
      srcB[r] = B + jc * ldb + kbeg + 2 * (q ^ ((j >> 1) & 7));
    }
    stepB = BK;
  }
  auto copy_one = [&](int stage, int slot, int c) {
    const int sc = stage < nst ? stage : nst - 1;
    double* base = lds + slot * SLOT;
    if (c < MBLK) hssk_glds16(srcA + sc * stepA + 64 * c, base + c * 1024 + wave * 128);
    else if (GEN) {}
    else if (TRANSB) hssk_glds16(srcB[c - MBLK] + sc * stepB, base + A_DBL + (c - MBLK) * 1024 + wave * 128);
    else hssk_glds16(srcB[c - MBLK] + sc * stepB, base + A_DBL + (wave + 8 * (c - MBLK)) * 128);
  };
  const int gen_dfirst = (int)kbeg - ((int)(jg0 + j0) + 127);
  auto gen_tau = [&](int i) {
    const int d = gen_dfirst + i;
    return TRANSB ? hssk_gen_eval(gen, 0, d) : hssk_gen_eval(gen, d, 0);
  };
  auto copy_stage = [&](int stage, int slot) {
#pragma unroll
    for (int c = 0; c < NCH; c++) copy_one(stage, slot, c);
  };

  int offA[MT], offB[NT][4];
#pragma unroll
  for (int a = 0; a < MT; a++) {
    const int il = wm + a * 16 + l15;
    offA[a] = hssk_opaque((il >> 6) * 1024 + ((l4 & 1) + 8 * (l4 >> 1)) * 64 + ((il & 63) ^ (16 * (l4 & 1))));
  }
#pragma unroll
  for (int b = 0; b < NT; b++) {
    const int jl = wn + b * 16 + l15;
    if (GEN) {
      const int o = hssk_opaque(A_DBL + (l4 & 1) + 8 * (l4 >> 1) + 127 - jl);
#pragma unroll
      for (int s = 0; s < 4; s++) offB[b][s] = o + 2 * s;
    } else if (KJ_IMAGE) {
      const int o = hssk_opaque(A_DBL + (jl >> 6) * 1024 + ((l4 & 1) + 8 * (l4 >> 1)) * 64 + ((jl & 63) ^ (16 * (l4 & 1))));
#pragma unroll
      for (int s = 0; s < 4; s++) offB[b][s] = o + s * 128;
    } else {
      const int h = (jl >> 1) & 7;
#pragma unroll
      for (int s = 0; s < 4; s++) offB[b][s] = hssk_opaque(A_DBL + jl * 16 + 2 * ((s + 4 * (l4 >> 1)) ^ h) + (l4 & 1));
    }
  }

  hssk_d4 acc[MT][NT];
#pragma unroll
  for (int a = 0; a < MT; a++)
#pragma unroll
    for (int b = 0; b < NT; b++) acc[a][b] = hssk_d4{0., 0., 0., 0.};
  double af[2][MT], bf[2][NT];
  auto frags = [&](int slot, int s, int set) {
    const double* base = lds + slot * SLOT;
#pragma unroll
    for (int a = 0; a < MT; a++) af[set][a] = base[offA[a] + s * 128];
#pragma unroll
    for (int b = 0; b < NT; b++) bf[set][b] = base[offB[b][s]];
  };
  auto mfmas = [&](int set) {
#pragma unroll
    for (int a = 0; a < MT; a++)
#pragma unroll
      for (int b = 0; b < NT; b++)
        acc[a][b] = hssk_mfma_f64_16x16x4(bf[set][b], af[set][a], acc[a][b]);
  };
  auto stage = [&](int st, auto slot_tag) {
    constexpr int S = decltype(slot_tag)::value;
    double gen_moved = 0.;
    if (GEN && wave < 2 && tid < 127) gen_moved = lds[((S + 1) % 3) * SLOT + A_DBL + tid + 16];
    frags(S, 1, 1);
    hssk_sched_barrier();
    mfmas(0);
    hssk_sched_barrier();
    if (GEN && wave < 2 && tid < 127) lds[((S + 2) % 3) * SLOT + A_DBL + tid] = gen_moved;
    if (GEN && wave == 2 + (st & 1)) lds[((S + 2) % 3) * SLOT + A_DBL + 127 + l15] = gen_tau(16 * (st + 2) + 127 + l15);
    hssk_sched_barrier();
    frags(S, 2, 0);
    hssk_sched_barrier();
    mfmas(1);
    hssk_sched_barrier();
    frags(S, 3, 1);
    hssk_sched_barrier();
    mfmas(0);
    hssk_sched_barrier();
    hssk_wait_glds<NCH>();
    hssk_wg_barrier();
    hssk_sched_barrier();
#pragma unroll
    for (int a = 0; a < MT; a++) {
#pragma unroll
      for (int b = 0; b < NT; b++) acc[a][b] = hssk_mfma_f64_16x16x4(bf[1][b], af[1][a], acc[a][b]);
      hssk_sched_barrier();
      if (a == 0) frags((S + 1) % 3, 0, 0);
      else if (a - 1 < NCH) copy_one(st + 3, S, a - 1);
      hssk_sched_barrier();
    }
#pragma unroll
    for (int c = MT - 1; c < NCH; c++) copy_one(st + 3, S, c);
    hssk_sched_barrier();
  };

  if (nst > 0) {
    copy_stage(0, 0);
    copy_stage(1, 1);
    copy_stage(2, 2);
    if (GEN && tid < 143) {
      lds[A_DBL + tid] = gen_tau(tid);
      lds[SLOT + A_DBL + tid] = gen_tau(16 + tid);
    }
    hssk_wait_glds<2 * NCH>();
    hssk_wg_barrier();
    frags(0, 0, 0);
    int st = 0;
    for (; st + 3 <= nst; st += 3) {
      stage(st, std::integral_constant<int, 0>());
      stage(st + 1, std::integral_constant<int, 1>());
      stage(st + 2, std::integral_constant<int, 2>());
    }
    if (st < nst) stage(st, std::integral_constant<int, 0>());
    if (st + 1 < nst) stage(st + 1, std::integral_constant<int, 1>());
    hssk_wait_glds<0>();
  }
  double* Pz = P + (long long)blockIdx.z * pstride;
#pragma unroll
  for (int a = 0; a < MT; a++)
#pragma unroll
    for (int b = 0; b < NT; b++)
#pragma unroll
      for (int r = 0; r < 4; r++) {
        const int gi = i0 + wm + a * 16 + l15;
        const long long gj = j0 + wn + b * 16 + l4 + 4 * r;
        Pz[gi + gj * ldp] = acc[a][b][r];
      }
  if (clk && threadIdx.x == 0) {
    const long long w1 = hssk_wallclock();
    if (blockIdx.x == 0 && blockIdx.y == 0 && blockIdx.z == 0) {
      clk[0] = hssk_clock() - t0_;
      clk[1] = w1 - w0_;
    }
    const long long fid = blockIdx.x + (long long)gridDim.x * (blockIdx.y + (long long)gridDim.y * blockIdx.z);
    long long* rec = clk + 4 + 4 * fid;
    rec[0] = w0_; rec[1] = w1; rec[2] = hssk_hwid(); rec[3] = bx;
  }
}

__global__ void dgemm_reduce_kernel(int m, long long n, const double* __restrict__ P, long long ldp,
                                    long long pstride, int nz, double alpha, double beta,
                                    double* __restrict__ C, long long ldc) {
  long long total = (long long)m * n;
  for (long long e = (long long)blockIdx.x * blockDim.x + threadIdx.x; e < total;
       e += (long long)gridDim.x * blockDim.x) {
    int i = (int)(e % m);
    long long j = e / m;
    double s = 0.;
    for (int z = 0; z < nz; z++) s += P[i + j * ldp + z * pstride];
    double* c = C + i + j * ldc;
    double v = alpha * s;
    if (beta != 0.) v += beta * (*c);
    *c = v;
  }
}

__global__ void dgemm_reduce_wide_kernel(int m, long long n, const double* __restrict__ P, long long ldp,
                                         long long pstride, int nz, double alpha, double beta,
                                         double* __restrict__ C, long long ldc) {
  HSSK_SHARED double s_part[256];
  const int el = threadIdx.x & 15, zl = threadIdx.x >> 4;
  const long long total = (long long)m * n;
  for (long long e0 = (long long)blockIdx.x * 16; e0 < total; e0 += (long long)gridDim.x * 16) {
    const long long e = e0 + el;
    const int i = (int)(e % m);
    const long long j = e / m;
    double s = 0.;
    if (e < total) {
      const double* p = P + i + j * ldp;
      for (int z = zl; z < nz; z += 16) s += p[z * pstride];
    }
    s_part[threadIdx.x] = s;
    __syncthreads();
    if (zl == 0 && e < total) {
      double t = 0.;
      for (int q = 0; q < 16; q++) t += s_part[el + 16 * q];
      double* c = C + i + j * ldc;
      double v = alpha * t;
      if (beta != 0.) v += beta * (*c);
      *c = v;
    }
    __syncthreads();
  }
}

template <int BM, bool FULL, int TAG>
void launch_dgemm(hssk_ctx* ctx, int transB, dim3 grid, int m, long long n, long long k, const double* A,
                  long long lda, const double* B, long long ldb, double* P, long long ldp, long long pstride,
                  long long kchunk, int jtile0, long long* clk) {
  if (grid.x == 0) return;
  if (transB)
    HSSK_LAUNCH((dgemm_kernel<BM, true, FULL, TAG>), grid, dim3(256), 0, ctx->stream, m, n, k, A, lda, B, ldb, P, ldp, pstride, kchunk, jtile0, clk);
  else
    HSSK_LAUNCH((dgemm_kernel<BM, false, FULL, TAG>), grid, dim3(256), 0, ctx->stream, m, n, k, A, lda, B, ldb, P, ldp, pstride, kchunk, jtile0, clk);
}

}

namespace {
template <bool FULL, int TAG>
void launch_bm(int BM, hssk_ctx* ctx, int transB, dim3 grid, int m, long long n, long long k, const double* A,
               long long lda, const double* B, long long ldb, double* P, long long ldp, long long pstride,
               long long kchunk, int jtile0, long long* clk) {
  if (BM == 192) launch_dgemm<192, FULL, TAG>(ctx, transB, grid, m, n, k, A, lda, B, ldb, P, ldp, pstride, kchunk, jtile0, clk);
  else if (BM == 128) launch_dgemm<128, FULL, TAG>(ctx, transB, grid, m, n, k, A, lda, B, ldb, P, ldp, pstride, kchunk, jtile0, clk);
  else launch_dgemm<64, FULL, TAG>(ctx, transB, grid, m, n, k, A, lda, B, ldb, P, ldp, pstride, kchunk, jtile0, clk);
}

constexpr int BN2 = 128;
inline size_t sketch_lds_bytes(int mblk) { return sizeof(double) * 3 * (size_t)(64 * mblk + BN2) * BK; }
template <int MBLK, int TAG>
void launch_sketch_m(hssk_ctx* ctx, int transB, dim3 grid, long long n, long long k, const double* A, long long lda,
                     const double* B, long long ldb, double* P, long long ldp, long long pstride, long long kchunk,
                     int jtile0, long long* clk, const hssk_gen* gen, long long jg0) {
  const size_t shm = sketch_lds_bytes(MBLK);
  const hssk_gen g0{0, 0, {0., 0., 0., 0.}};
  if (gen) {
    if (transB) HSSK_LAUNCH((sketch_kernel<MBLK, true, TAG, true>), grid, dim3(512), shm, ctx->stream, n, k, A, lda, B, ldb, P, ldp, pstride, kchunk, jtile0, clk, *gen, jg0);
    else HSSK_LAUNCH((sketch_kernel<MBLK, false, TAG, true>), grid, dim3(512), shm, ctx->stream, n, k, A, lda, B, ldb, P, ldp, pstride, kchunk, jtile0, clk, *gen, jg0);
  } else {
    if (transB) HSSK_LAUNCH((sketch_kernel<MBLK, true, TAG, false>), grid, dim3(512), shm, ctx->stream, n, k, A, lda, B, ldb, P, ldp, pstride, kchunk, jtile0, clk, g0, jg0);
    else HSSK_LAUNCH((sketch_kernel<MBLK, false, TAG, false>), grid, dim3(512), shm, ctx->stream, n, k, A, lda, B, ldb, P, ldp, pstride, kchunk, jtile0, clk, g0, jg0);
  }
}
template <int MBLK>
bool sketch_prepare_m() {
  static const bool ok = [] {
    try {
      const size_t b = sketch_lds_bytes(MBLK);
      if (b > hssk_rt::max_lds_per_workgroup()) return false;
      hssk_rt::allow_dynamic_lds(sketch_kernel<MBLK, true, 0, false>, b);
      hssk_rt::allow_dynamic_lds(sketch_kernel<MBLK, false, 0, false>, b);
      hssk_rt::allow_dynamic_lds(sketch_kernel<MBLK, true, 1, false>, b);
      hssk_rt::allow_dynamic_lds(sketch_kernel<MBLK, false, 1, false>, b);
      hssk_rt::allow_dynamic_lds(sketch_kernel<MBLK, true, 0, true>, b);
      hssk_rt::allow_dynamic_lds(sketch_kernel<MBLK, false, 0, true>, b);
      hssk_rt::allow_dynamic_lds(sketch_kernel<MBLK, true, 1, true>, b);
      hssk_rt::allow_dynamic_lds(sketch_kernel<MBLK, false, 1, true>, b);
      return true;
    } catch (const std::exception&) {
      return false;
    }
  }();
  return ok;
}
inline bool sketch_prepare(int BM) {
  return BM == 192 ? sketch_prepare_m<3>() : (BM == 128 ? sketch_prepare_m<2>() : sketch_prepare_m<1>());
}
template <int TAG>
void launch_sketch(int BM, hssk_ctx* ctx, int transB, dim3 grid, long long n, long long k, const double* A, long long lda,
                   const double* B, long long ldb, double* P, long long ldp, long long pstride, long long kchunk,
                   int jtile0, long long* clk, const hssk_gen* gen, long long jg0) {
  if (grid.x == 0) return;
  if (BM == 192) launch_sketch_m<3, TAG>(ctx, transB, grid, n, k, A, lda, B, ldb, P, ldp, pstride, kchunk, jtile0, clk, gen, jg0);
  else if (BM == 128) launch_sketch_m<2, TAG>(ctx, transB, grid, n, k, A, lda, B, ldb, P, ldp, pstride, kchunk, jtile0, clk, gen, jg0);
  else launch_sketch_m<1, TAG>(ctx, transB, grid, n, k, A, lda, B, ldb, P, ldp, pstride, kchunk, jtile0, clk, gen, jg0);
}
}

static void dgemm_impl(hssk_ctx* ctx, int transB, int m, long long n, long long k, double alpha, const double* A, long long lda,
                       const double* B, long long ldb, const hssk_gen* gen, long long jg0, double beta, double* C, long long ldc) {
  if (m <= 0 || n <= 0) return;
  const int BM = m > 128 ? 192 : (m > 64 ? 128 : 64);
  const unsigned gm = (unsigned)((m + BM - 1) / BM);
  const long long ksteps = (k + BK - 1) / BK;
  const bool aligned = (m % BM == 0) && (k % BK == 0) && (lda % 2 == 0) && (gen || ldb % 2 == 0) &&
                       (((size_t)A | (gen ? (size_t)0 : (size_t)B)) % 16 == 0);
  static const int cus = hssk_rt::cu_count();
  const bool force_v1 = [] { const char* e = std::getenv("HSSK_DGEMM_V1"); return e && std::atoi(e) != 0; }();
  const bool v2 = aligned && (gen || !force_v1) && k > 0 && n >= BN2 && sketch_prepare(BM);
  if (gen && !v2) {
    const long long nb_max = std::max<long long>(64, std::min<long long>(1024, (long long)(size_t(1) << 28) / std::max<long long>(k, 1)));
    const long long ldg = k + (k & 1);
    for (long long c0 = 0; c0 < n; c0 += nb_max) {
      const long long nb = std::min(nb_max, n - c0);
      double* G = ctx->gen_block(sizeof(double) * (size_t)ldg * nb);
      if (hssk_gen_fill(ctx, gen, G, k, nb, ldg, 0, jg0 + c0, transB)) throw std::runtime_error(hssk_last_error());
      dgemm_impl(ctx, 0, m, nb, k, alpha, A, lda, G, ldg, nullptr, 0, beta, C + c0 * ldc, ldc);
    }
    return;
  }
  const int BNt = v2 ? BN2 : BN;
  static const bool no_fold = [] { const char* e = std::getenv("HSSK_DGEMM_NO_FOLD"); return e && std::atoi(e) != 0; }();
  const bool fold_edge = v2 && !no_fold && n % BNt != 0 && n % 2 == 0;
  const unsigned gn_full = aligned ? (unsigned)(n / BNt) + (fold_edge ? 1u : 0u) : 0u;
  const long long edge_col0 = std::min<long long>(n, (long long)gn_full * BNt);
  const unsigned gn_edge = (unsigned)((n - edge_col0 + BN - 1) / BN);
  const long long slots = v2 ? cus : 2LL * cus;
  struct Group { long long col0 = 0, ntiles = 0; int split = 1; long long kchunk = BK; int nz = 0; double* P = nullptr; long long cols = 0, vcols = 0; };
  auto chunk_of = [&](int split) {
    long long c = ((ksteps + split - 1) / split) * BK;
    return c > 0 ? c : (long long)BK;
  };
  auto max_split = [&]() { return (int)std::max<long long>(1, std::min<long long>(256, ksteps / 24)); };
  auto one_round_split = [&](long long tiles) {
    if (tiles <= 0 || k <= 0) return 1;
    return (int)std::max<long long>(1, std::min<long long>(max_split(), slots / tiles));
  };
  Group gmain, gtail, gedge;
  if (gn_full) {
    const long long T = (long long)gm * gn_full;
    const double epi = 3.0, red = 0.0067 * (BNt / BN);
    double best = 1e300;
    int best_s = 1;
    long long best_main = T;
    const int sp_min = (int)std::min<long long>(std::min(max_split(), 64), (ksteps + 1023) / 1024);
    for (int sp = std::max(1, sp_min); sp <= std::min(max_split(), 64); sp++) {
      const long long r = (T * sp) / slots;
      long long tm = r > 0 ? std::min<long long>(T, (r * slots) / sp) : 0;
      if (gm > 1) tm = T;
      const long long tt = T - tm;
      double cost = 0.;
      if (tm) cost += (double)((tm * sp + slots - 1) / slots) * ((double)(ksteps + sp - 1) / sp + epi) + red * sp * (double)tm;
      if (tt) {
        const int st = one_round_split(tt);
        cost += (double)((tt * st + slots - 1) / slots) * ((double)(ksteps + st - 1) / st + epi) + red * st * (double)tt + 2.0;
      }
      if (cost < best - 1e-9) { best = cost; best_s = sp; best_main = tm; }
    }
    if (k <= 0) { best_s = 1; best_main = T; }
    if (const char* e = std::getenv("HSSK_DGEMM_SPLIT")) {
      const int sp = std::max(1, std::min(max_split(), std::atoi(e)));
      const long long r = (T * sp) / slots;
      best_s = sp;
      best_main = (gm > 1 || r == 0) ? T : std::min<long long>(T, (r * slots) / sp);
    }
    gmain.col0 = 0; gmain.ntiles = gm > 1 ? gn_full : best_main; gmain.split = best_s; gmain.cols = gmain.ntiles * BNt;
    gtail.col0 = gmain.cols; gtail.ntiles = gn_full - gmain.ntiles; gtail.split = one_round_split(gtail.ntiles); gtail.cols = gtail.ntiles * BNt;
  }
  gedge.col0 = edge_col0; gedge.ntiles = gn_edge; gedge.split = one_round_split((long long)gm * gn_edge); gedge.cols = n - edge_col0;
  const long long ldp = m;
  size_t ptot = 0;
  for (Group* g : {&gmain, &gtail, &gedge}) {
    if (!g->ntiles) continue;
    g->vcols = std::min(g->cols, n - g->col0);
    g->kchunk = chunk_of(g->split);
    g->nz = (int)std::max<long long>(1, (k + g->kchunk - 1) / g->kchunk);
    ptot += (size_t)ldp * g->cols * g->nz;
  }
  const size_t ntrace = gmain.ntiles ? (size_t)gmain.ntiles * gm * gmain.nz : 0;
  double* P = ctx->scratch(sizeof(double) * (ptot + 4 + 4 * ntrace));
  long long* clk = (long long*)(P + ptot);
  {
    double* q = P;
    for (Group* g : {&gmain, &gtail, &gedge}) {
      if (!g->ntiles) continue;
      g->P = q;
      q += (size_t)ldp * g->cols * g->nz;
    }
  }
  auto shifted = [&](const Group& g) { return g.P - g.col0 * ldp; };
  const Group* timed = gmain.ntiles ? &gmain : (gtail.ntiles ? &gtail : &gedge);
  auto bracket = [&](const Group* g, auto&& launch) {
    if (!g->ntiles) return;
    if (g == timed) hssk_rt::event_record(ctx->ev0, ctx->stream);
    launch();
    if (g == timed) hssk_rt::event_record(ctx->ev1, ctx->stream);
  };
  auto grid_of = [&](const Group& g) { return dim3((unsigned)g.ntiles, gm, (unsigned)g.nz); };
  if (gen && gedge.ntiles) {
    const long long ldg = k + (k & 1);
    double* G = ctx->gen_block(sizeof(double) * (size_t)ldg * gedge.cols);
    if (hssk_gen_fill(ctx, gen, G, k, gedge.cols, ldg, 0, jg0 + gedge.col0, transB)) throw std::runtime_error(hssk_last_error());
    const double* Gs = G - gedge.col0 * ldg;
    bracket(&gedge, [&] { launch_bm<false, 0>(BM, ctx, 0, grid_of(gedge), m, n, k, A, lda, Gs, ldg, shifted(gedge), ldp, ldp * gedge.cols, gedge.kchunk, (int)(gedge.col0 / BN), nullptr); });
  } else
  bracket(&gedge, [&] { launch_bm<false, 0>(BM, ctx, transB, grid_of(gedge), m, n, k, A, lda, B, ldb, shifted(gedge), ldp, ldp * gedge.cols, gedge.kchunk, (int)(gedge.col0 / BN), nullptr); });
  if (v2) {
    bracket(&gtail, [&] { launch_sketch<1>(BM, ctx, transB, grid_of(gtail), n, k, A, lda, B, ldb, shifted(gtail), ldp, ldp * gtail.cols, gtail.kchunk, (int)(gtail.col0 / BN2), nullptr, gen, jg0); });
    bracket(&gmain, [&] { launch_sketch<0>(BM, ctx, transB, grid_of(gmain), n, k, A, lda, B, ldb, shifted(gmain), ldp, ldp * gmain.cols, gmain.kchunk, (int)(gmain.col0 / BN2), clk, gen, jg0); });
  } else {
    bracket(&gtail, [&] { launch_bm<true, 1>(BM, ctx, transB, grid_of(gtail), m, n, k, A, lda, B, ldb, shifted(gtail), ldp, ldp * gtail.cols, gtail.kchunk, (int)(gtail.col0 / BN), nullptr); });
    bracket(&gmain, [&] { launch_bm<true, 0>(BM, ctx, transB, grid_of(gmain), m, n, k, A, lda, B, ldb, shifted(gmain), ldp, ldp * gmain.cols, gmain.kchunk, (int)(gmain.col0 / BN), clk); });
  }
  ctx->d_clk = gmain.ntiles ? clk : nullptr;
  ctx->dgemm_trace_wgs = (long long)ntrace;
  ctx->dgemm_timed = true;
  ctx->dgemm_timed_flops = 2.0 * (double)m * (double)timed->vcols * (double)k;
  for (const Group* g : {&gmain, &gtail, &gedge}) {
    if (!g->ntiles) continue;
    long long total = (long long)m * g->vcols;
    unsigned rb = (unsigned)std::min<long long>((total + 255) / 256, 4096);
    if (g->nz >= 32 && total <= 65536)
      HSSK_LAUNCH(dgemm_reduce_wide_kernel, dim3((unsigned)((total + 15) / 16)), dim3(256), 0, ctx->stream, m, g->vcols, (const double*)g->P, ldp, ldp * g->cols, g->nz, alpha, beta, C + g->col0 * ldc, ldc);
    else
      HSSK_LAUNCH(dgemm_reduce_kernel, dim3(rb), dim3(256), 0, ctx->stream, m, g->vcols, (const double*)g->P, ldp, ldp * g->cols, g->nz, alpha, beta, C + g->col0 * ldc, ldc);
  }
  hssk_rt::check_launch();
}

extern "C" int hssk_dgemm(hssk_ctx* ctx, int transB, int m, long long n, long long k, double alpha,
                          const double* A, long long lda, const double* B, long long ldb, double beta,
                          double* C, long long ldc) {
  HSSK_API_BEGIN
  dgemm_impl(ctx, transB, m, n, k, alpha, A, lda, B, ldb, nullptr, 0, beta, C, ldc);
  HSSK_API_END
}

extern "C" int hssk_sketch_gen(hssk_ctx* ctx, const hssk_gen* g, int transG, int m, long long n, long long k, long long j0,
                               double alpha, const double* A, long long lda, double beta, double* C, long long ldc) {
  HSSK_API_BEGIN
  if (!g || (g->kind != HSSK_GEN_TOEPLITZ && g->kind != HSSK_GEN_TOEPLITZ_UPPER)) throw std::invalid_argument("hssk_sketch_gen: unknown generator kind");
  if (k > 0x7fffffffLL || j0 + n > 0x7fffffffLL) throw std::invalid_argument("hssk_sketch_gen: indices beyond 2^31");
  dgemm_impl(ctx, transG, m, n, k, alpha, A, lda, nullptr, 0, g, j0, beta, C, ldc);
  HSSK_API_END
}
```

### strumpack_amd/csrc/kernels/hssk_internal.h

```cpp
#pragma once
#include <functional>
#include <vector>
#include <algorithm>
#include <utility>
#include <cstring>
#include <stdexcept>
#include <string>

#include "hssk.h"
#include "hssk_rt.h"

namespace hssk_rec {
extern thread_local std::vector<std::function<void()>>* sink;
}

struct hssk_plan {
  std::vector<std::function<void()>> launches;
  struct Block { char* dev; char* shadow; size_t size; };
  std::vector<Block> blocks;
  size_t off = 0;
  char* alloc(size_t bytes, char** shadow) {
    const size_t need = (bytes + 255) & ~size_t(255);
    if (blocks.empty() || off + need > blocks.back().size) {
      const size_t sz = std::max<size_t>(need, size_t(1) << 20);
      blocks.push_back(Block{(char*)hssk_rt::dev_malloc(sz), (char*)hssk_rt::pinned_malloc(sz), sz});
      off = 0;
    }
    char* p = blocks.back().dev + off;
    *shadow = blocks.back().shadow + off;
    off += need;
    return p;
  }
  ~hssk_plan() { for (auto& b : blocks) { hssk_rt::dev_free(b.dev); hssk_rt::pinned_free(b.shadow); } }
};

struct hssk_uploader;
struct hssk_ctx {
  int device = 0;
  hssk_rt::stream_t stream{};
  char* h_ring = nullptr;
  char* d_ring = nullptr;
  size_t ring_bytes = 0, ring_off = 0;
  size_t zero_copy_bytes = 0;
  hssk_rt::event_t ev0{}, ev1{};
  hssk_rt::event_t ev_sync{};
  hssk_rt::stream_t side{}, main_saved{};
  hssk_rt::event_t ev_fork{}, ev_join{};
  bool on_side = false, side_made = false;
  bool require_mma = false;
  bool dgemm_timed = false;
  double dgemm_timed_flops = 0.;
  struct TimedBracket { hssk_rt::event_t a, b; double flops; };
  std::vector<TimedBracket> dgemm_deferred;
  long long dgemm_trace_wgs = 0;
  long long* d_clk = nullptr;
  double* d_scratch = nullptr;
  struct hssk_uploader* uploader = nullptr;
  int* d_sweep_flags = nullptr;
  int* h_sweep_err = nullptr;
  std::vector<std::pair<hssk_rt::event_t, hssk_rt::event_t>> watch[8];
  std::vector<hssk_rt::event_t> watch_free;
  bool watch_open[8] = {false, false, false, false, false, false, false, false};
  size_t sweep_cap = size_t(1) << 20;
  size_t scratch_bytes = 0;

  hssk_plan* recording = nullptr;
  void* stage(const void* host, size_t bytes) {
    if (recording) {
      char* shadow = nullptr;
      char* p = recording->alloc(bytes, &shadow);
      std::memcpy(shadow, host, bytes);
      hssk_rt::h2d(p, shadow, bytes, stream);
      return p;
    }
    size_t need = (bytes + 255) & ~size_t(255);
    if (need > ring_bytes) throw std::runtime_error("hssk: descriptor batch exceeds staging ring");
    if (ring_off + need > ring_bytes) {
      hssk_rt::sync(stream);
      if (side_made) {
        hssk_rt::sync(side);
        if (on_side) hssk_rt::sync(main_saved);
      }
      ring_off = 0;
    }
    std::memcpy(h_ring + ring_off, host, bytes);
    void* d;
    if (bytes <= zero_copy_bytes) {
      d = h_ring + ring_off;
    } else {
      hssk_rt::h2d(d_ring + ring_off, h_ring + ring_off, bytes, stream);
      d = d_ring + ring_off;
    }
    ring_off += need;
    return d;
  }
  double* d_aux = nullptr;
  size_t aux_bytes = 0;
  void sync_all() {
    hssk_rt::sync(stream);
    if (side_made) {
      hssk_rt::sync(side);
      if (on_side) hssk_rt::sync(main_saved);
    }
  }
  double* aux(size_t bytes) {
    if (bytes > aux_bytes) {
      sync_all();
      hssk_rt::dev_free(d_aux);
      d_aux = (double*)hssk_rt::dev_malloc(bytes);
      aux_bytes = bytes;
    }
    return d_aux;
  }
  double* d_gen = nullptr;
  size_t gen_bytes = 0;
  double* gen_block(size_t bytes) {
    if (bytes > gen_bytes) {
      sync_all();
      hssk_rt::dev_free(d_gen);
      d_gen = (double*)hssk_rt::dev_malloc(bytes);
      gen_bytes = bytes;
    }
    return d_gen;
  }
  double* scratch(size_t bytes) {
    if (bytes > scratch_bytes) {
      sync_all();
      hssk_rt::dev_free(d_scratch);
      d_scratch = (double*)hssk_rt::dev_malloc(bytes);
      scratch_bytes = bytes;
    }
    return d_scratch;
  }
};

void hssk_set_error(const std::string& msg);

#define HSSK_UNSUPPORTED(msg) do { hssk_set_error(std::string(__func__) + ": " + (msg)); return 2; } while (0)
#define HSSK_API_BEGIN try {
#define HSSK_API_END                 \
  return 0;                          \
  }                                  \
  catch (const std::exception& e) {  \
    hssk_set_error(e.what());        \
    return 1;                        \
  }
```

### strumpack_amd/hssk.py

```python
import ctypes as C

import numpy as np

c_dp = C.POINTER(C.c_double)
c_ip = C.POINTER(C.c_int)


class GemmDesc(C.Structure):
    _fields_ = [("A", C.c_void_p), ("B", C.c_void_p), ("C", C.c_void_p),
                ("m", C.c_int), ("n", C.c_int), ("k", C.c_int),
                ("lda", C.c_int), ("ldb", C.c_int), ("ldc", C.c_int),
                ("transA", C.c_int), ("transB", C.c_int),
                ("alpha", C.c_double), ("beta", C.c_double)]


class LeafUpdateDesc(C.Structure):
    _fields_ = [("R", C.c_void_p), ("D", C.c_void_p), ("Sr", C.c_void_p), ("Sc", C.c_void_p),
                ("d", C.c_int), ("m", C.c_int), ("ldr", C.c_int), ("ldd", C.c_int), ("lds", C.c_int)]


class KernelSpec(C.Structure):
    _fields_ = [("X", C.c_void_p), ("n", C.c_longlong), ("d", C.c_int), ("type", C.c_int), ("p", C.c_int),
                ("h", C.c_double), ("lam", C.c_double)]


class KevalDesc(C.Structure):
    _fields_ = [("ri", C.c_void_p), ("ci", C.c_void_p), ("out", C.c_void_p),
                ("nr", C.c_int), ("nc", C.c_int), ("ldo", C.c_int), ("r0", C.c_int), ("c0", C.c_int)]


class ColsetDesc(C.Structure):
    _fields_ = [("src0", C.c_void_p), ("src1", C.c_void_p), ("n0", C.c_int), ("n1", C.c_int), ("lo", C.c_int), ("hi", C.c_int),
                ("out", C.c_void_p), ("count", C.c_void_p), ("n0_dev", C.c_void_p), ("n1_dev", C.c_void_p)]


class ColGatherDesc(C.Structure):
    _fields_ = [("src", C.c_void_p), ("dst", C.c_void_p), ("idx", C.c_void_p),
                ("rows", C.c_int), ("ncols", C.c_int), ("lds", C.c_int), ("ldd", C.c_int),
                ("scatter", C.c_int)]


class RowGatherDesc(C.Structure):
    _fields_ = [("src", C.c_void_p), ("dst", C.c_void_p), ("idx", C.c_void_p),
                ("nrows", C.c_int), ("cols", C.c_int), ("lds", C.c_int), ("ldd", C.c_int),
                ("scatter", C.c_int), ("accumulate", C.c_int)]


class ElemDesc(C.Structure):
    _fields_ = [("A", C.c_void_p), ("lda", C.c_longlong), ("I", C.c_void_p), ("J", C.c_void_p),
                ("i0", C.c_int), ("j0", C.c_int), ("B", C.c_void_p),
                ("m", C.c_int), ("n", C.c_int), ("ldb", C.c_int), ("transpose", C.c_int),
                ("rlo", C.c_int), ("rhi", C.c_int), ("clo", C.c_int), ("chi", C.c_int)]


class TransposeDesc(C.Structure):
    _fields_ = [("src", C.c_void_p), ("dst", C.c_void_p),
                ("rows", C.c_int), ("cols", C.c_int), ("lds", C.c_int), ("ldd", C.c_int)]


class IdDesc(C.Structure):
    _fields_ = [("W", C.c_void_p), ("ldw", C.c_int), ("d", C.c_int), ("m", C.c_int),
                ("rtol", C.c_double), ("atol", C.c_double), ("max_rank", C.c_int),
                ("perm", C.c_void_p), ("rank", C.c_void_p), ("work", C.c_void_p),
                ("src", C.c_void_p), ("lds", C.c_int), ("defer_x", C.c_int)]


class CombineDesc(C.Structure):
    _fields_ = [("G0", C.c_void_p), ("G1", C.c_void_p), ("ldg", C.c_int), ("gsplit", C.c_int), ("gidx", C.c_void_p),
                ("M0", C.c_void_p), ("M1", C.c_void_p), ("ldm", C.c_int), ("msplit", C.c_int), ("midx", C.c_void_p),
                ("C", C.c_void_p), ("csj", C.c_int), ("csk", C.c_int), ("alpha", C.c_double),
                ("out", C.c_void_p), ("ldo", C.c_int), ("rows", C.c_int), ("J", C.c_int), ("K", C.c_int)]


class UlvSplitDesc(C.Structure):
    _fields_ = [("D", C.c_void_p), ("ldd", C.c_int), ("m", C.c_int), ("r", C.c_int), ("perm", C.c_void_p),
                ("X", C.c_void_p), ("ldx", C.c_int), ("W1", C.c_void_p), ("ldw", C.c_int), ("W0t", C.c_void_p), ("ldt", C.c_int)]


class TpqrDesc(C.Structure):
    _fields_ = [("R1", C.c_void_p), ("ld1", C.c_int), ("R2", C.c_void_p), ("ld2", C.c_int), ("m", C.c_int)]


class XsolveDesc(C.Structure):
    _fields_ = [("W", C.c_void_p), ("ldw", C.c_int), ("rank", C.c_int), ("m", C.c_int),
                ("X", C.c_void_p), ("ldx", C.c_int), ("solved", C.c_int)]


class PcholDesc(C.Structure):
    _fields_ = [("G", C.c_void_p), ("ldg", C.c_int), ("m", C.c_int), ("rtol", C.c_double), ("atol", C.c_double),
                ("max_rank", C.c_int), ("perm", C.c_void_p), ("rank", C.c_void_p), ("R", C.c_void_p), ("ldr", C.c_int)]


class SumDesc(C.Structure):
    _fields_ = [("P", C.c_void_p), ("stride", C.c_longlong), ("n", C.c_longlong), ("count", C.c_int), ("out", C.c_void_p)]


class GramDesc(C.Structure):
    _fields_ = [("W", C.c_void_p), ("ldw", C.c_int), ("rows", C.c_int), ("m", C.c_int), ("G", C.c_void_p), ("ldg", C.c_int)]


class GramGenDesc(C.Structure):
    _fields_ = [("ri", C.c_void_p), ("r0", C.c_int), ("ci", C.c_void_p), ("c0", C.c_int), ("rows", C.c_int), ("m", C.c_int),
                ("G", C.c_void_p), ("ldg", C.c_int)]


class QrDesc(C.Structure):
    _fields_ = [("A", C.c_void_p), ("lda", C.c_int), ("rows", C.c_int), ("cols", C.c_int),
                ("Q", C.c_void_p), ("ldq", C.c_int), ("nq", C.c_int),
                ("rdiag", C.c_void_p), ("work", C.c_void_p), ("stair", C.c_int),
                ("stop_rel", C.c_double), ("stop_abs", C.c_double), ("r_only", C.c_int)]


class TrsmDesc(C.Structure):
    _fields_ = [("T", C.c_void_p), ("B", C.c_void_p), ("n", C.c_int), ("nrhs", C.c_int),
                ("ldt", C.c_int), ("ldb", C.c_int), ("lower", C.c_int), ("transT", C.c_int),
                ("unit", C.c_int), ("Tinv", C.c_void_p)]


class TrtriDesc(C.Structure):
    _fields_ = [("R", C.c_void_p), ("Tinv", C.c_void_p), ("n", C.c_int), ("ldr", C.c_int), ("mode", C.c_int)]


class LuDesc(C.Structure):
    _fields_ = [("A", C.c_void_p), ("n", C.c_int), ("lda", C.c_int), ("piv", C.c_void_p),
                ("info", C.c_void_p)]


class LuSolveDesc(C.Structure):
    _fields_ = [("LU", C.c_void_p), ("piv", C.c_void_p), ("B", C.c_void_p),
                ("n", C.c_int), ("nrhs", C.c_int), ("lda", C.c_int), ("ldb", C.c_int)]


class NormDesc(C.Structure):
    _fields_ = [("P", C.c_void_p), ("rows", C.c_int), ("cols", C.c_int), ("ld", C.c_int),
                ("out", C.c_void_p)]


class ShiftDesc(C.Structure):
    _fields_ = [("A", C.c_void_p), ("n", C.c_int), ("lda", C.c_int)]


class Gen(C.Structure):
    _fields_ = [("kind", C.c_int), ("reserved", C.c_int), ("p", C.c_double * 4)]


HSSK_SYMBOLS = [
    "hssk_ctx_create", "hssk_ctx_destroy", "hssk_ctx_stream", "hssk_sync", "hssk_last_error",
    "hssk_malloc", "hssk_free", "hssk_memcpy_h2d", "hssk_memcpy_d2h", "hssk_last_dgemm_ms", "hssk_last_dgemm_flops", "hssk_last_dgemm_trace",
    "hssk_fill_toeplitz", "hssk_randn", "hssk_dgemm", "hssk_gemm_vbatched", "hssk_gather_cols",
    "hssk_gather_rows", "hssk_gather_elems", "hssk_transpose", "hssk_id_vbatched",
    "hssk_qr_vbatched", "hssk_trsm_vbatched", "hssk_getrf_vbatched", "hssk_getrs_vbatched",
    "hssk_sumsq_vbatched", "hssk_shift_diag", "hssk_mfma_f64_peak_tflops", "hssk_memcpy_d2d",
    "hssk_memcpy2d_h2d", "hssk_memcpy2d_d2h", "hssk_memset_zero", "hssk_is_device_pointer",
    "hssk_basis_dense", "hssk_mfma_f64_probe", "hssk_last_dgemm_clock_ghz", "hssk_leaf_update_vbatched", "hssk_formq_vbatched",
    "hssk_kernel_eval_vbatched", "hssk_knn", "hssk_kernel_predict", "hssk_copy_triu",
    "hssk_laswp_vbatched", "hssk_shift_diag_cplx", "hssk_upload_async", "hssk_h2d_block_async", "hssk_h2d_bytes_async", "hssk_expand_image", "hssk_copy_fence", "hssk_compute_fence", "hssk_compute_mark", "hssk_copy_wait", "hssk_id_xsolve_vbatched", "hssk_id_solves_inline", "hssk_gather_combine", "hssk_ulv_split", "hssk_tpqr_vbatched", "hssk_fill_toeplitz_block", "hssk_sum_slabs", "hssk_ulv_fwd_sweep", "hssk_ulv_bwd_sweep", "hssk_apply_sweep", "hssk_sweep_status", "hssk_sweep_arm", "hssk_trtri_diag_vbatched", "hssk_sjlt_dense", "hssk_sjlt_sketch",
    "hssk_plan_begin", "hssk_plan_end", "hssk_plan_replay", "hssk_plan_destroy", "hssk_plan_size",
    "hssk_sketch_gen", "hssk_gen_elems", "hssk_gen_fill", "hssk_colsets", "hssk_colsets_max_universe",
    "hssk_cluster_median", "hssk_pchol_id_vbatched", "hssk_pchol_id_max_m", "hssk_pchol_id_rank_cap", "hssk_sum_partials", "hssk_gram_vbatched", "hssk_gram_gen_vbatched", "hssk_gram_gen_supported",
    "hssk_sgemm_sketch", "hssk_narrow_f32", "hssk_gather_elems_f32",
    "hssk_kernel_predict_f32", "hssk_kernel_predict_splits",
]


class DevArray:

    def __init__(self, hk, shape, dtype=np.float64):
        self.hk, self.shape, self.dtype = hk, tuple(shape), np.dtype(dtype)
        self.nbytes = int(np.prod(self.shape)) * self.dtype.itemsize
        self.ptr = hk.lib.hssk_malloc(max(self.nbytes, 8))
        if not self.ptr:
            raise MemoryError(hk.error())

    def free(self):
        if self.ptr:
            self.hk.lib.hssk_free(self.ptr)
            self.ptr = None

    def __del__(self):
        try:
            self.free()
        except Exception:
            pass

    def get(self):
        out = np.empty(self.shape, dtype=self.dtype, order="F")
        if self.nbytes:
            self.hk.check(self.hk.lib.hssk_memcpy_d2h(self.hk.ctx, out.ctypes.data, self.ptr, self.nbytes))
        return out

    def set(self, arr):
        a = np.asfortranarray(arr, dtype=self.dtype)
        assert a.shape == self.shape
        if self.nbytes:
            self.hk.check(self.hk.lib.hssk_memcpy_h2d(self.hk.ctx, self.ptr, a.ctypes.data, self.nbytes))
        return self

    def at(self, *idx):
        off, stride = 0, 1
        for i, n in zip(idx, self.shape):
            off += i * stride
            stride *= n
        return self.ptr + off * self.dtype.itemsize


class Hssk:
    def __init__(self, path, device=0):
        self.lib = L = C.CDLL(path)
        L.hssk_malloc.restype = C.c_void_p
        L.hssk_malloc.argtypes = [C.c_longlong]
        L.hssk_free.argtypes = [C.c_void_p]
        L.hssk_last_error.restype = C.c_char_p
        L.hssk_ctx_create.argtypes = [C.POINTER(C.c_void_p), C.c_int]
        L.hssk_ctx_destroy.argtypes = [C.c_void_p]
        L.hssk_ctx_stream.restype = C.c_void_p
        L.hssk_ctx_stream.argtypes = [C.c_void_p]
        L.hssk_sync.argtypes = [C.c_void_p]
        L.hssk_memcpy_h2d.argtypes = [C.c_void_p, C.c_void_p, C.c_void_p, C.c_longlong]
        L.hssk_memcpy_d2h.argtypes = [C.c_void_p, C.c_void_p, C.c_void_p, C.c_longlong]
        L.hssk_memcpy_d2d.argtypes = [C.c_void_p, C.c_void_p, C.c_void_p, C.c_longlong]
        L.hssk_memset_zero.argtypes = [C.c_void_p, C.c_void_p, C.c_longlong]
        for f in ("hssk_memcpy2d_h2d", "hssk_memcpy2d_d2h"):
            getattr(L, f).argtypes = [C.c_void_p, C.c_void_p, C.c_longlong, C.c_void_p, C.c_longlong,
                                      C.c_longlong, C.c_longlong]
        L.hssk_is_device_pointer.argtypes = [C.c_void_p]
        L.hssk_last_dgemm_clock_ghz.restype = C.c_double
        L.hssk_last_dgemm_clock_ghz.argtypes = [C.c_void_p]
        L.hssk_last_dgemm_ms.restype = C.c_float
        L.hssk_last_dgemm_ms.argtypes = [C.c_void_p]
        L.hssk_last_dgemm_trace.restype = C.c_longlong
        L.hssk_last_dgemm_trace.argtypes = [C.c_void_p, C.c_void_p, C.c_longlong]
        L.hssk_last_dgemm_flops.restype = C.c_double
        L.hssk_last_dgemm_flops.argtypes = [C.c_void_p]
        L.hssk_fill_toeplitz.argtypes = [C.c_void_p, C.c_void_p, C.c_int, C.c_longlong, C.c_char]
        L.hssk_fill_toeplitz_block.argtypes = [C.c_void_p, C.c_void_p, C.c_int, C.c_int, C.c_longlong, C.c_int, C.c_int, C.c_char]
        L.hssk_sum_slabs.argtypes = [C.c_void_p, C.c_void_p, C.c_longlong, C.c_longlong, C.c_int, C.c_void_p]
        L.hssk_upload_async.argtypes = [C.c_void_p, C.c_void_p, C.c_void_p, C.c_longlong]
        L.hssk_h2d_block_async.argtypes = [C.c_void_p, C.c_void_p, C.c_longlong, C.c_void_p, C.c_longlong, C.c_longlong, C.c_longlong]
        L.hssk_copy_fence.argtypes = [C.c_void_p]
        L.hssk_compute_fence.argtypes = [C.c_void_p]
        L.hssk_h2d_bytes_async.argtypes = [C.c_void_p, C.c_void_p, C.c_longlong, C.c_void_p, C.c_longlong, C.c_longlong, C.c_longlong]
        L.hssk_expand_image.argtypes = [C.c_void_p, C.c_void_p, C.c_longlong, C.c_void_p, C.c_longlong, C.c_longlong, C.c_longlong, C.c_int]
        L.hssk_compute_mark.argtypes = [C.c_void_p, C.c_int]
        L.hssk_copy_wait.argtypes = [C.c_void_p, C.c_int]
        L.hssk_sweep_status.argtypes = [C.c_void_p]
        L.hssk_randn.argtypes = [C.c_void_p, C.c_void_p, C.c_int, C.c_longlong, C.c_longlong,
                                 C.c_int, C.c_longlong, C.c_ulonglong]
        L.hssk_dgemm.argtypes = [C.c_void_p, C.c_int, C.c_int, C.c_longlong, C.c_longlong,
                                 C.c_double, C.c_void_p, C.c_longlong, C.c_void_p, C.c_longlong,
                                 C.c_double, C.c_void_p, C.c_longlong]
        L.hssk_sgemm_sketch.argtypes = [C.c_void_p, C.c_int, C.c_int, C.c_longlong, C.c_longlong,
                                        C.c_double, C.c_void_p, C.c_longlong, C.c_void_p, C.c_longlong,
                                        C.c_double, C.c_void_p, C.c_longlong]
        L.hssk_narrow_f32.argtypes = [C.c_void_p, C.c_void_p, C.c_longlong, C.c_void_p, C.c_longlong, C.c_longlong, C.c_longlong]
        for name in ("hssk_gemm_vbatched", "hssk_gather_cols", "hssk_gather_rows",
                     "hssk_gather_elems", "hssk_gather_elems_f32", "hssk_transpose", "hssk_id_vbatched", "hssk_qr_vbatched",
                     "hssk_trsm_vbatched", "hssk_getrf_vbatched", "hssk_getrs_vbatched",
                     "hssk_sumsq_vbatched", "hssk_leaf_update_vbatched", "hssk_formq_vbatched",
                     "hssk_id_xsolve_vbatched", "hssk_gather_combine", "hssk_ulv_split", "hssk_tpqr_vbatched"):
            getattr(L, name).argtypes = [C.c_void_p, C.c_void_p, C.c_int]
        L.hssk_sketch_gen.argtypes = [C.c_void_p, C.c_void_p, C.c_int, C.c_int, C.c_longlong, C.c_longlong, C.c_longlong,
                                      C.c_double, C.c_void_p, C.c_longlong, C.c_double, C.c_void_p, C.c_longlong]
        L.hssk_gen_elems.argtypes = [C.c_void_p, C.c_void_p, C.c_void_p, C.c_int]
        L.hssk_gen_fill.argtypes = [C.c_void_p, C.c_void_p, C.c_void_p, C.c_longlong, C.c_longlong, C.c_longlong, C.c_longlong,
                                    C.c_longlong, C.c_int]
        L.hssk_id_solves_inline.argtypes = [C.c_int, C.c_int]
        L.hssk_shift_diag.argtypes = [C.c_void_p, C.c_void_p, C.c_int, C.c_double]
        L.hssk_kernel_eval_vbatched.argtypes = [C.c_void_p, C.c_void_p, C.c_void_p, C.c_int]
        L.hssk_knn.argtypes = [C.c_void_p, C.c_void_p, C.c_int, C.c_int, C.c_int, C.c_int, C.c_int, C.c_void_p]
        L.hssk_kernel_predict.argtypes = [C.c_void_p, C.c_void_p, C.c_void_p, C.c_void_p, C.c_int, C.c_void_p]
        L.hssk_kernel_predict_f32.argtypes = [C.c_void_p, C.c_void_p, C.c_longlong, C.c_int, C.c_int, C.c_int, C.c_double,
                                              C.c_void_p, C.c_void_p, C.c_int, C.c_void_p, C.c_void_p]
        L.hssk_kernel_predict_splits.argtypes = [C.c_longlong, C.c_int]
        L.hssk_colsets.argtypes = [C.c_void_p, C.c_void_p, C.c_int, C.c_int]
        L.hssk_cluster_median.argtypes = [C.c_void_p, C.c_void_p, C.c_int, C.c_int, C.c_int, C.c_int, C.c_void_p, C.c_void_p]
        for fn in ("hssk_pchol_id_vbatched", "hssk_sum_partials", "hssk_gram_vbatched"):
            getattr(L, fn).argtypes = [C.c_void_p, C.c_void_p, C.c_int]
        L.hssk_pchol_id_rank_cap.argtypes = [C.c_int]
        L.hssk_gram_gen_vbatched.argtypes = [C.c_void_p, C.c_void_p, C.c_void_p, C.c_int]
        L.hssk_gram_gen_supported.argtypes = [C.c_void_p, C.c_int]
        L.hssk_colsets_max_universe.argtypes = []
        L.hssk_colsets_max_universe.restype = C.c_longlong
        L.hssk_sjlt_dense.argtypes = [C.c_void_p, C.c_void_p, C.c_int, C.c_longlong, C.c_longlong, C.c_void_p, C.c_int]
        L.hssk_sjlt_sketch.argtypes = [C.c_void_p, C.c_int, C.c_longlong, C.c_longlong, C.c_void_p, C.c_longlong,
                                       C.c_void_p, C.c_int, C.c_int, C.c_void_p, C.c_longlong]
        L.hssk_mfma_f64_peak_tflops.restype = C.c_double
        L.hssk_mfma_f64_peak_tflops.argtypes = [C.c_void_p, C.c_int]
        L.hssk_mfma_f64_probe.argtypes = [C.c_void_p, C.c_int, C.c_int, C.c_int, C.POINTER(C.c_double)]
        ctx = C.c_void_p()
        if L.hssk_ctx_create(C.byref(ctx), device):
            raise RuntimeError(self.error())
        self.ctx = ctx

    def error(self):
        return self.lib.hssk_last_error().decode()

    def check(self, rc):
        if rc:
            raise RuntimeError(self.error())

    def close(self):
        if self.ctx:
            self.lib.hssk_ctx_destroy(self.ctx)
            self.ctx = None

    def sync(self):
        self.check(self.lib.hssk_sync(self.ctx))

    def empty(self, shape, dtype=np.float64):
        return DevArray(self, shape, dtype)

    def array(self, arr, dtype=None):
        a = np.asarray(arr)
        d = DevArray(self, a.shape, dtype or a.dtype)
        return d.set(a)

    def kernel_predict_f32(self, X, w, T, ktype, h, p=1, stats=False):
        X = np.ascontiguousarray(X, dtype=np.float32)
        T = np.ascontiguousarray(T, dtype=np.float32)
        w = np.ascontiguousarray(w, dtype=np.float32)
        (n, d), m = X.shape, T.shape[0]
        dX, dT, dw, dp = (self.array(X.ravel()), self.array(T.ravel()), self.array(w), self.empty((m,), np.float32))
        st = np.zeros(6, dtype=np.int64)
        self.check(self.lib.hssk_kernel_predict_f32(self.ctx, dX.ptr, n, d, ktype, p, h, dw.ptr, dT.ptr, m, dp.ptr,
                                                    st.ctypes.data if stats else None))
        out = dp.get()
        for a in (dX, dT, dw, dp):
            a.free()
        return (out, st) if stats else out

    def batch(self, fn_name, descs):
        if not descs:
            return
        arr = (type(descs[0]) * len(descs))(*descs)
        self.check(getattr(self.lib, fn_name)(self.ctx, arr, len(descs)))
```

Baseline: 69520.

## Merge sketch main/tail groups into one launch and overlap split-K reduction on side stream

```diff
diff --git a/include/hssk.h b/include/hssk.h
--- a/include/hssk.h
+++ b/include/hssk.h
@@ -64,6 +64,7 @@
 int hssk_dgemm_timing_defer(hssk_ctx* ctx);
 int hssk_dgemm_timing_collect(hssk_ctx* ctx, double* ms, double* flops, int* launches);
 long long hssk_last_dgemm_trace(hssk_ctx* ctx, long long* out, long long max_wgs);
+int hssk_last_dgemm_groups(hssk_ctx* ctx, long long out[12]);
 double hssk_last_dgemm_clock_ghz(hssk_ctx* ctx);
 
 int hssk_fill_toeplitz(hssk_ctx* ctx, double* A, int n, long long lda, char kind);
@@ -74,6 +75,8 @@
 int hssk_dgemm(hssk_ctx* ctx, int transB, int m, long long n, long long k, double alpha,
                const double* A, long long lda, const double* B, long long ldb, double beta,
                double* C, long long ldc);
+int hssk_dgemm_fold_next(hssk_ctx* ctx);
+int hssk_dgemm_fold_join(hssk_ctx* ctx);
 
 int hssk_sgemm_sketch(hssk_ctx* ctx, int transB, int m, long long n, long long k, double alpha,
                       const double* A, long long lda,
diff --git a/strumpack_amd/csrc/host/hss_sources.cpp b/strumpack_amd/csrc/host/hss_sources.cpp
--- a/strumpack_amd/csrc/host/hss_sources.cpp
+++ b/strumpack_amd/csrc/host/hss_sources.cpp
@@ -46,6 +46,7 @@
         }
       }
     } else if (nloc > 0) {
+      if (!H.o_.symmetric) ck(hssk_dgemm_fold_next(H.ctx_));
       ck(hssk_dgemm(H.ctx_, 1, dn, nloc, N, 1.0, H.Rt_ + r0, H.dcap_, dA + j0, lda, 0.0, H.Srt_ + r0 + j0 * H.dcap_, H.dcap_));
       ck(hssk_dgemm_timing_defer(H.ctx_));
       if (H.o_.symmetric) {
@@ -54,6 +55,7 @@
       } else {
         ck(hssk_dgemm(H.ctx_, 0, dn, nloc, N, 1.0, H.Rt_ + r0, H.dcap_, dA + j0 * lda, lda, 0.0, H.Sct_ + r0 + j0 * H.dcap_, H.dcap_));
         ck(hssk_dgemm_timing_defer(H.ctx_));
+        ck(hssk_dgemm_fold_join(H.ctx_));
       }
     }
     if (H.o_.world > 1 && !H.dist_subtree_) {
@@ -153,17 +155,20 @@
     const Node& c = H.nodes_[single ? 0 : H.cut_nodes_[H.o_.rank]];
     const long long j0 = c.lo, nloc = c.m;
     auto timed = [&] { ck(hssk_dgemm_timing_defer(H.ctx_)); };
+    ck(hssk_dgemm_fold_next(H.ctx_));
     ck(hssk_dgemm(H.ctx_, 0, dn, nloc, N, 1.0, H.Rt_ + r0, H.dcap_, dCols, ldc, 0.0, H.Sct_ + r0 + j0 * H.dcap_, H.dcap_));
     timed();
     if (dRows) {
       ck(hssk_dgemm(H.ctx_, 1, dn, nloc, N, 1.0, H.Rt_ + r0, H.dcap_, dRows, ldr, 0.0, H.Srt_ + r0 + j0 * H.dcap_, H.dcap_));
       timed();
+      ck(hssk_dgemm_fold_join(H.ctx_));
     } else {
       H.tmp_->rewind();
       double* P = H.tmp_->dbl((size_t)dn * N);
       double* mineP = H.tmp_->dbl((size_t)dn * nloc);
       ck(hssk_dgemm(H.ctx_, 1, dn, N, nloc, 1.0, H.Rt_ + r0 + j0 * H.dcap_, H.dcap_, dCols, ldc, 0.0, P, dn));
       timed();
+      ck(hssk_dgemm_fold_join(H.ctx_));
       const double tc = now();
       std::vector<long long> offs(H.o_.world), counts(H.o_.world);
       for (int g = 0; g < H.o_.world; g++) {
@@ -437,6 +442,7 @@
     const long long nloc = j1 - j0;
     auto timed = [&] { ck(hssk_dgemm_timing_defer(H.ctx_)); };
     if (nloc > 0) {
+      if (!H.o_.symmetric) ck(hssk_dgemm_fold_next(H.ctx_));
       ck(hssk_sketch_gen(H.ctx_, &g, 1, dn, nloc, N, j0, 1.0, H.Rt_ + r0, H.dcap_, 0.0, H.Srt_ + r0 + j0 * H.dcap_, H.dcap_));
       timed();
       if (H.o_.symmetric) {
@@ -445,6 +451,7 @@
       } else {
         ck(hssk_sketch_gen(H.ctx_, &g, 0, dn, nloc, N, j0, 1.0, H.Rt_ + r0, H.dcap_, 0.0, H.Sct_ + r0 + j0 * H.dcap_, H.dcap_));
         timed();
+        ck(hssk_dgemm_fold_join(H.ctx_));
       }
     }
     if (H.o_.world > 1 && !H.dist_subtree_) {
diff --git a/strumpack_amd/csrc/kernels/hssk_ctx.hip b/strumpack_amd/csrc/kernels/hssk_ctx.hip
--- a/strumpack_amd/csrc/kernels/hssk_ctx.hip
+++ b/strumpack_amd/csrc/kernels/hssk_ctx.hip
@@ -251,6 +251,9 @@
 void hssk_ctx_destroy(hssk_ctx* c) {
   if (!c) return;
   try { hssk_rt::sync(c->stream); } catch (...) {}
+  if (c->fold_busy[0] || c->fold_busy[1]) { try { hssk_rt::sync(c->side); } catch (...) {} }
+  c->fold_busy[0] = c->fold_busy[1] = c->fold_armed = false;
+  c->fold_sel = 0;
   {
     std::lock_guard<std::mutex> g(g_pool_mu);
     if (g_pool.size() < 8) {
@@ -272,6 +275,8 @@
   hssk_rt::pinned_free(c->h_ring);
   hssk_rt::dev_free(c->d_ring);
   hssk_rt::dev_free(c->d_scratch);
+  hssk_rt::dev_free(c->d_scratch2);
+  if (c->fold_events) { hssk_rt::event_destroy(c->ev_fold); hssk_rt::event_destroy(c->ev_fold_done[0]); hssk_rt::event_destroy(c->ev_fold_done[1]); }
   hssk_rt::dev_free(c->d_aux);
   hssk_rt::dev_free(c->d_gen);
   delete c->uploader;
@@ -300,12 +305,7 @@
 int hssk_side_begin(hssk_ctx* c) {
   HSSK_API_BEGIN
   if (c->on_side) throw std::logic_error("hssk_side_begin: already on the side stream");
-  if (!c->side_made) {
-    c->side = hssk_rt::stream_create();
-    c->ev_fork = hssk_rt::event_create();
-    c->ev_join = hssk_rt::event_create();
-    c->side_made = true;
-  }
+  c->make_side();
   auto f = [c]() {
     hssk_rt::event_record(c->ev_fork, c->stream);
     hssk_rt::stream_wait_event(c->side, c->ev_fork);
diff --git a/strumpack_amd/csrc/kernels/hssk_dgemm.hip b/strumpack_amd/csrc/kernels/hssk_dgemm.hip
--- a/strumpack_amd/csrc/kernels/hssk_dgemm.hip
+++ b/strumpack_amd/csrc/kernels/hssk_dgemm.hip
@@ -210,13 +210,24 @@
   }
 }
 
+struct sketch_group {
+  int wgs, ntiles, jtile0;
+  long long kchunk, pstride;
+  double* P;
+};
 template <int MBLK, bool TRANSB, int TAG = 0, bool GEN = false>
 __global__ __launch_bounds__(512, 2) void sketch_kernel(long long n, long long k, const double* __restrict__ A, long long lda,
-                                                        const double* __restrict__ B, long long ldb,
-                                                        double* __restrict__ P, long long ldp, long long pstride,
-                                                        long long kchunk, int jtile0, long long* __restrict__ clk,
+                                                        const double* __restrict__ B, long long ldb, long long ldp, int gm,
+                                                        sketch_group g0, sketch_group g1, long long* __restrict__ clk,
                                                         hssk_gen gen, long long jg0) {
   const long long t0_ = clk ? hssk_clock() : 0, w0_ = clk ? hssk_wallclock() : 0;
+  int fid = blockIdx.x;
+  const bool in_tail = fid >= g0.wgs;
+  if (in_tail) fid -= g0.wgs;
+  const int ntiles = in_tail ? g1.ntiles : g0.ntiles, jtile0 = in_tail ? g1.jtile0 : g0.jtile0;
+  const long long kchunk = in_tail ? g1.kchunk : g0.kchunk, pstride = in_tail ? g1.pstride : g0.pstride;
+  double* __restrict__ P = in_tail ? g1.P : g0.P;
+  const int fyz = fid / ntiles, by = fyz % gm, bz = fyz / gm;
   constexpr int BM = 64 * MBLK, BN2 = 128;
   constexpr int WM = BM / 2, MT = WM / 16, NT = 2;
   constexpr int A_DBL = BM * BK, B_DBL = BN2 * BK, SLOT = A_DBL + B_DBL;
@@ -226,14 +237,14 @@
 
   const int tid = threadIdx.x, lane = tid & 63, wave = hssk_uniform(tid >> 6);
   const int l15 = lane & 15, l4 = lane >> 4;
-  int bx = blockIdx.x;
+  int bx = fid - fyz * ntiles;
   {
-    const int nx = gridDim.x, x = bx & 7, q = nx >> 3, r = nx & 7;
+    const int nx = ntiles, x = bx & 7, q = nx >> 3, r = nx & 7;
     bx = x * q + (x < r ? x : r) + (bx >> 3);
   }
   const long long j0 = (long long)(bx + jtile0) * BN2;
-  const int i0 = blockIdx.y * BM;
-  const long long kbeg = (long long)blockIdx.z * kchunk;
+  const int i0 = by * BM;
+  const long long kbeg = (long long)bz * kchunk;
   const long long kend = kbeg + kchunk < k ? kbeg + kchunk : k;
   const int nst = (int)((kend - kbeg) / BK);
   const int wm = (wave & 1) * WM, wn = (wave >> 1) * 32;
@@ -377,7 +388,7 @@
     if (st + 1 < nst) stage(st + 1, std::integral_constant<int, 1>());
     hssk_wait_glds<0>();
   }
-  double* Pz = P + (long long)blockIdx.z * pstride;
+  double* Pz = P + (long long)bz * pstride;
 #pragma unroll
   for (int a = 0; a < MT; a++)
 #pragma unroll
@@ -390,13 +401,12 @@
       }
   if (clk && threadIdx.x == 0) {
     const long long w1 = hssk_wallclock();
-    if (blockIdx.x == 0 && blockIdx.y == 0 && blockIdx.z == 0) {
+    if (blockIdx.x == 0) {
       clk[0] = hssk_clock() - t0_;
       clk[1] = w1 - w0_;
     }
-    const long long fid = blockIdx.x + (long long)gridDim.x * (blockIdx.y + (long long)gridDim.y * blockIdx.z);
-    long long* rec = clk + 4 + 4 * fid;
-    rec[0] = w0_; rec[1] = w1; rec[2] = hssk_hwid(); rec[3] = bx;
+    long long* rec = clk + 4 + 4 * (long long)blockIdx.x;
+    rec[0] = w0_; rec[1] = w1; rec[2] = hssk_hwid(); rec[3] = bx + jtile0;
   }
 }
 
@@ -471,18 +481,19 @@
 
 constexpr int BN2 = 128;
 inline size_t sketch_lds_bytes(int mblk) { return sizeof(double) * 3 * (size_t)(64 * mblk + BN2) * BK; }
-template <int MBLK, int TAG>
-void launch_sketch_m(hssk_ctx* ctx, int transB, dim3 grid, long long n, long long k, const double* A, long long lda,
-                     const double* B, long long ldb, double* P, long long ldp, long long pstride, long long kchunk,
-                     int jtile0, long long* clk, const hssk_gen* gen, long long jg0) {
+template <int MBLK>
+void launch_sketch_m(hssk_rt::stream_t stream, int transB, long long n, long long k, const double* A, long long lda,
+                     const double* B, long long ldb, long long ldp, int gm, const sketch_group& g0, const sketch_group& g1,
+                     long long* clk, const hssk_gen* gen, long long jg0) {
   const size_t shm = sketch_lds_bytes(MBLK);
-  const hssk_gen g0{0, 0, {0., 0., 0., 0.}};
+  const hssk_gen gz{0, 0, {0., 0., 0., 0.}};
+  const dim3 grid((unsigned)(g0.wgs + g1.wgs));
   if (gen) {
-    if (transB) HSSK_LAUNCH((sketch_kernel<MBLK, true, TAG, true>), grid, dim3(512), shm, ctx->stream, n, k, A, lda, B, ldb, P, ldp, pstride, kchunk, jtile0, clk, *gen, jg0);
-    else HSSK_LAUNCH((sketch_kernel<MBLK, false, TAG, true>), grid, dim3(512), shm, ctx->stream, n, k, A, lda, B, ldb, P, ldp, pstride, kchunk, jtile0, clk, *gen, jg0);
+    if (transB) HSSK_LAUNCH((sketch_kernel<MBLK, true, 0, true>), grid, dim3(512), shm, stream, n, k, A, lda, B, ldb, ldp, gm, g0, g1, clk, *gen, jg0);
+    else HSSK_LAUNCH((sketch_kernel<MBLK, false, 0, true>), grid, dim3(512), shm, stream, n, k, A, lda, B, ldb, ldp, gm, g0, g1, clk, *gen, jg0);
   } else {
-    if (transB) HSSK_LAUNCH((sketch_kernel<MBLK, true, TAG, false>), grid, dim3(512), shm, ctx->stream, n, k, A, lda, B, ldb, P, ldp, pstride, kchunk, jtile0, clk, g0, jg0);
-    else HSSK_LAUNCH((sketch_kernel<MBLK, false, TAG, false>), grid, dim3(512), shm, ctx->stream, n, k, A, lda, B, ldb, P, ldp, pstride, kchunk, jtile0, clk, g0, jg0);
+    if (transB) HSSK_LAUNCH((sketch_kernel<MBLK, true, 0, false>), grid, dim3(512), shm, stream, n, k, A, lda, B, ldb, ldp, gm, g0, g1, clk, gz, jg0);
+    else HSSK_LAUNCH((sketch_kernel<MBLK, false, 0, false>), grid, dim3(512), shm, stream, n, k, A, lda, B, ldb, ldp, gm, g0, g1, clk, gz, jg0);
   }
 }
 template <int MBLK>
@@ -493,12 +504,8 @@
       if (b > hssk_rt::max_lds_per_workgroup()) return false;
       hssk_rt::allow_dynamic_lds(sketch_kernel<MBLK, true, 0, false>, b);
       hssk_rt::allow_dynamic_lds(sketch_kernel<MBLK, false, 0, false>, b);
-      hssk_rt::allow_dynamic_lds(sketch_kernel<MBLK, true, 1, false>, b);
-      hssk_rt::allow_dynamic_lds(sketch_kernel<MBLK, false, 1, false>, b);
       hssk_rt::allow_dynamic_lds(sketch_kernel<MBLK, true, 0, true>, b);
       hssk_rt::allow_dynamic_lds(sketch_kernel<MBLK, false, 0, true>, b);
-      hssk_rt::allow_dynamic_lds(sketch_kernel<MBLK, true, 1, true>, b);
-      hssk_rt::allow_dynamic_lds(sketch_kernel<MBLK, false, 1, true>, b);
       return true;
     } catch (const std::exception&) {
       return false;
@@ -509,14 +516,13 @@
 inline bool sketch_prepare(int BM) {
   return BM == 192 ? sketch_prepare_m<3>() : (BM == 128 ? sketch_prepare_m<2>() : sketch_prepare_m<1>());
 }
-template <int TAG>
-void launch_sketch(int BM, hssk_ctx* ctx, int transB, dim3 grid, long long n, long long k, const double* A, long long lda,
-                   const double* B, long long ldb, double* P, long long ldp, long long pstride, long long kchunk,
-                   int jtile0, long long* clk, const hssk_gen* gen, long long jg0) {
-  if (grid.x == 0) return;
-  if (BM == 192) launch_sketch_m<3, TAG>(ctx, transB, grid, n, k, A, lda, B, ldb, P, ldp, pstride, kchunk, jtile0, clk, gen, jg0);
-  else if (BM == 128) launch_sketch_m<2, TAG>(ctx, transB, grid, n, k, A, lda, B, ldb, P, ldp, pstride, kchunk, jtile0, clk, gen, jg0);
-  else launch_sketch_m<1, TAG>(ctx, transB, grid, n, k, A, lda, B, ldb, P, ldp, pstride, kchunk, jtile0, clk, gen, jg0);
+inline void launch_sketch(int BM, hssk_rt::stream_t stream, int transB, long long n, long long k, const double* A, long long lda,
+                          const double* B, long long ldb, long long ldp, int gm, const sketch_group& g0, const sketch_group& g1,
+                          long long* clk, const hssk_gen* gen, long long jg0) {
+  if (g0.wgs + g1.wgs <= 0) return;
+  if (BM == 192) launch_sketch_m<3>(stream, transB, n, k, A, lda, B, ldb, ldp, gm, g0, g1, clk, gen, jg0);
+  else if (BM == 128) launch_sketch_m<2>(stream, transB, n, k, A, lda, B, ldb, ldp, gm, g0, g1, clk, gen, jg0);
+  else launch_sketch_m<1>(stream, transB, n, k, A, lda, B, ldb, ldp, gm, g0, g1, clk, gen, jg0);
 }
 }
 
@@ -548,7 +554,10 @@
   const unsigned gn_full = aligned ? (unsigned)(n / BNt) + (fold_edge ? 1u : 0u) : 0u;
   const long long edge_col0 = std::min<long long>(n, (long long)gn_full * BNt);
   const unsigned gn_edge = (unsigned)((n - edge_col0 + BN - 1) / BN);
-  const long long slots = v2 ? cus : 2LL * cus;
+  auto env_ll = [](const char* name) { const char* e = std::getenv(name); return e ? std::atoll(e) : 0LL; };
+  const bool two_launch = env_ll("HSSK_DGEMM_TWO_LAUNCH") != 0;
+  const bool merged = v2 && !two_launch;
+  const long long slots = env_ll("HSSK_DGEMM_SLOTS") > 0 ? env_ll("HSSK_DGEMM_SLOTS") : (v2 ? cus : 2LL * cus);
   struct Group { long long col0 = 0, ntiles = 0; int split = 1; long long kchunk = BK; int nz = 0; double* P = nullptr; long long cols = 0, vcols = 0; };
   auto chunk_of = [&](int split) {
     long long c = ((ksteps + split - 1) / split) * BK;
@@ -559,10 +568,14 @@
     if (tiles <= 0 || k <= 0) return 1;
     return (int)std::max<long long>(1, std::min<long long>(max_split(), slots / tiles));
   };
+  const double epi = 3.0, red = 0.0067 * (BNt / BN);
+  const int tail_fixed = [&] { const char* e = std::getenv("HSSK_DGEMM_TAIL_SPLIT"); return e ? std::max(0, std::min(max_split(), std::atoi(e))) : 0; }();
+  auto tail_split = [&](long long tiles) {
+    return (tail_fixed > 0 && tiles > 0 && k > 0) ? tail_fixed : one_round_split(tiles);
+  };
   Group gmain, gtail, gedge;
   if (gn_full) {
     const long long T = (long long)gm * gn_full;
-    const double epi = 3.0, red = 0.0067 * (BNt / BN);
     double best = 1e300;
     int best_s = 1;
     long long best_main = T;
@@ -588,7 +601,7 @@
       best_main = (gm > 1 || r == 0) ? T : std::min<long long>(T, (r * slots) / sp);
     }
     gmain.col0 = 0; gmain.ntiles = gm > 1 ? gn_full : best_main; gmain.split = best_s; gmain.cols = gmain.ntiles * BNt;
-    gtail.col0 = gmain.cols; gtail.ntiles = gn_full - gmain.ntiles; gtail.split = one_round_split(gtail.ntiles); gtail.cols = gtail.ntiles * BNt;
+    gtail.col0 = gmain.cols; gtail.ntiles = gn_full - gmain.ntiles; gtail.split = tail_split(gtail.ntiles); gtail.cols = gtail.ntiles * BNt;
   }
   gedge.col0 = edge_col0; gedge.ntiles = gn_edge; gedge.split = one_round_split((long long)gm * gn_edge); gedge.cols = n - edge_col0;
   const long long ldp = m;
@@ -600,8 +613,14 @@
     g->nz = (int)std::max<long long>(1, (k + g->kchunk - 1) / g->kchunk);
     ptot += (size_t)ldp * g->cols * g->nz;
   }
-  const size_t ntrace = gmain.ntiles ? (size_t)gmain.ntiles * gm * gmain.nz : 0;
-  double* P = ctx->scratch(sizeof(double) * (ptot + 4 + 4 * ntrace));
+  auto wgs_of = [&](const Group& g) { return (long long)g.ntiles * gm * g.nz; };
+  if (v2 && wgs_of(gmain) + wgs_of(gtail) > 0x7fffffffLL) throw std::invalid_argument("hssk_dgemm: more than 2^31 workgroups");
+  const size_t ntrace = (size_t)wgs_of(gmain) + (merged ? (size_t)wgs_of(gtail) : 0);
+  const bool fold = ctx->fold_armed && !two_launch && !ctx->on_side && !hssk_rec::sink;
+  ctx->fold_armed = false;
+  const int region = ctx->fold_sel;
+  const size_t pbytes = sizeof(double) * (ptot + 4 + 4 * ntrace);
+  double* P = region ? ctx->scratch2(pbytes) : ctx->scratch(pbytes);
   long long* clk = (long long*)(P + ptot);
   {
     double* q = P;
@@ -613,11 +632,15 @@
   }
   auto shifted = [&](const Group& g) { return g.P - g.col0 * ldp; };
   const Group* timed = gmain.ntiles ? &gmain : (gtail.ntiles ? &gtail : &gedge);
+  const bool timed_merged = merged && (gmain.ntiles || gtail.ntiles);
+  int launches = 0;
   auto bracket = [&](const Group* g, auto&& launch) {
     if (!g->ntiles) return;
-    if (g == timed) hssk_rt::event_record(ctx->ev0, ctx->stream);
+    const bool t = g == timed && !timed_merged;
+    if (t) hssk_rt::event_record(ctx->ev0, ctx->stream);
     launch();
-    if (g == timed) hssk_rt::event_record(ctx->ev1, ctx->stream);
+    launches++;
+    if (t) hssk_rt::event_record(ctx->ev1, ctx->stream);
   };
   auto grid_of = [&](const Group& g) { return dim3((unsigned)g.ntiles, gm, (unsigned)g.nz); };
   if (gen && gedge.ntiles) {
@@ -629,24 +652,64 @@
   } else
   bracket(&gedge, [&] { launch_bm<false, 0>(BM, ctx, transB, grid_of(gedge), m, n, k, A, lda, B, ldb, shifted(gedge), ldp, ldp * gedge.cols, gedge.kchunk, (int)(gedge.col0 / BN), nullptr); });
   if (v2) {
-    bracket(&gtail, [&] { launch_sketch<1>(BM, ctx, transB, grid_of(gtail), n, k, A, lda, B, ldb, shifted(gtail), ldp, ldp * gtail.cols, gtail.kchunk, (int)(gtail.col0 / BN2), nullptr, gen, jg0); });
-    bracket(&gmain, [&] { launch_sketch<0>(BM, ctx, transB, grid_of(gmain), n, k, A, lda, B, ldb, shifted(gmain), ldp, ldp * gmain.cols, gmain.kchunk, (int)(gmain.col0 / BN2), clk, gen, jg0); });
+    auto sk_group = [&](const Group& g) {
+      sketch_group s{0, 0, 0, (long long)BK, 0, nullptr};
+      if (g.ntiles) s = sketch_group{(int)wgs_of(g), (int)g.ntiles, (int)(g.col0 / BN2), g.kchunk, ldp * g.cols, shifted(g)};
+      return s;
+    };
+    const sketch_group none = sk_group(Group());
+    if (merged) {
+      if (timed_merged) {
+        hssk_rt::event_record(ctx->ev0, ctx->stream);
+        launch_sketch(BM, ctx->stream, transB, n, k, A, lda, B, ldb, ldp, (int)gm, sk_group(gmain), sk_group(gtail), clk, gen, jg0);
+        launches++;
+        hssk_rt::event_record(ctx->ev1, ctx->stream);
+      }
+    } else {
+      bracket(&gtail, [&] { launch_sketch(BM, ctx->stream, transB, n, k, A, lda, B, ldb, ldp, (int)gm, sk_group(gtail), none, nullptr, gen, jg0); });
+      bracket(&gmain, [&] { launch_sketch(BM, ctx->stream, transB, n, k, A, lda, B, ldb, ldp, (int)gm, sk_group(gmain), none, clk, gen, jg0); });
+    }
   } else {
     bracket(&gtail, [&] { launch_bm<true, 1>(BM, ctx, transB, grid_of(gtail), m, n, k, A, lda, B, ldb, shifted(gtail), ldp, ldp * gtail.cols, gtail.kchunk, (int)(gtail.col0 / BN), nullptr); });
     bracket(&gmain, [&] { launch_bm<true, 0>(BM, ctx, transB, grid_of(gmain), m, n, k, A, lda, B, ldb, shifted(gmain), ldp, ldp * gmain.cols, gmain.kchunk, (int)(gmain.col0 / BN), clk); });
   }
-  ctx->d_clk = gmain.ntiles ? clk : nullptr;
-  ctx->dgemm_trace_wgs = (long long)ntrace;
+  const bool traced = ntrace > 0 && (timed_merged || gmain.ntiles);
+  ctx->d_clk = traced ? clk : nullptr;
+  ctx->dgemm_trace_wgs = traced ? (long long)ntrace : 0;
   ctx->dgemm_timed = true;
-  ctx->dgemm_timed_flops = 2.0 * (double)m * (double)timed->vcols * (double)k;
+  ctx->dgemm_timed_flops = 2.0 * (double)m * (double)(timed_merged ? gmain.vcols + gtail.vcols : timed->vcols) * (double)k;
+  {
+    long long* o = ctx->dgemm_groups;
+    const Group* gs[3] = {&gmain, &gtail, &gedge};
+    for (int q = 0; q < 3; q++) { o[3 * q] = gs[q]->ntiles; o[3 * q + 1] = gs[q]->ntiles ? gs[q]->nz : 0; o[3 * q + 2] = gs[q]->col0; }
+    o[9] = launches; o[10] = region; o[11] = fold ? 1 : 0;
+  }
+  hssk_rt::stream_t rs = ctx->stream;
+  if (fold) {
+    ctx->make_side();
+    if (!ctx->fold_events) {
+      ctx->ev_fold = hssk_rt::event_create();
+      ctx->ev_fold_done[0] = hssk_rt::event_create();
+      ctx->ev_fold_done[1] = hssk_rt::event_create();
+      ctx->fold_events = true;
+    }
+    hssk_rt::event_record(ctx->ev_fold, ctx->stream);
+    hssk_rt::stream_wait_event(ctx->side, ctx->ev_fold);
+    rs = ctx->side;
+  }
   for (const Group* g : {&gmain, &gtail, &gedge}) {
     if (!g->ntiles) continue;
     long long total = (long long)m * g->vcols;
     unsigned rb = (unsigned)std::min<long long>((total + 255) / 256, 4096);
     if (g->nz >= 32 && total <= 65536)
-      HSSK_LAUNCH(dgemm_reduce_wide_kernel, dim3((unsigned)((total + 15) / 16)), dim3(256), 0, ctx->stream, m, g->vcols, (const double*)g->P, ldp, ldp * g->cols, g->nz, alpha, beta, C + g->col0 * ldc, ldc);
+      HSSK_LAUNCH(dgemm_reduce_wide_kernel, dim3((unsigned)((total + 15) / 16)), dim3(256), 0, rs, m, g->vcols, (const double*)g->P, ldp, ldp * g->cols, g->nz, alpha, beta, C + g->col0 * ldc, ldc);
     else
-      HSSK_LAUNCH(dgemm_reduce_kernel, dim3(rb), dim3(256), 0, ctx->stream, m, g->vcols, (const double*)g->P, ldp, ldp * g->cols, g->nz, alpha, beta, C + g->col0 * ldc, ldc);
+      HSSK_LAUNCH(dgemm_reduce_kernel, dim3(rb), dim3(256), 0, rs, m, g->vcols, (const double*)g->P, ldp, ldp * g->cols, g->nz, alpha, beta, C + g->col0 * ldc, ldc);
+  }
+  if (fold) {
+    hssk_rt::event_record(ctx->ev_fold_done[region], ctx->side);
+    ctx->fold_busy[region] = true;
+    ctx->fold_sel = region ^ 1;
   }
   hssk_rt::check_launch();
 }
@@ -667,3 +730,27 @@
   dgemm_impl(ctx, transG, m, n, k, alpha, A, lda, nullptr, 0, g, j0, beta, C, ldc);
   HSSK_API_END
 }
+
+extern "C" int hssk_dgemm_fold_next(hssk_ctx* ctx) {
+  HSSK_API_BEGIN
+  const char* e = std::getenv("HSSK_DGEMM_FOLD");
+  ctx->fold_armed = !(e && std::atoi(e) == 0);
+  HSSK_API_END
+}
+extern "C" int hssk_dgemm_fold_join(hssk_ctx* ctx) {
+  HSSK_API_BEGIN
+  ctx->fold_armed = false;
+  for (int r = 0; r < 2; r++)
+    if (ctx->fold_busy[r]) {
+      if (ctx->on_side) throw std::logic_error("hssk_dgemm_fold_join: on the side stream");
+      hssk_rt::stream_wait_event(ctx->stream, ctx->ev_fold_done[r]);
+      ctx->fold_busy[r] = false;
+    }
+  ctx->fold_sel = 0;
+  HSSK_API_END
+}
+extern "C" int hssk_last_dgemm_groups(hssk_ctx* ctx, long long out[12]) {
+  HSSK_API_BEGIN
+  for (int q = 0; q < 12; q++) out[q] = ctx->dgemm_groups[q];
+  HSSK_API_END
+}
diff --git a/strumpack_amd/csrc/kernels/hssk_internal.h b/strumpack_amd/csrc/kernels/hssk_internal.h
--- a/strumpack_amd/csrc/kernels/hssk_internal.h
+++ b/strumpack_amd/csrc/kernels/hssk_internal.h
@@ -55,6 +55,13 @@
   long long dgemm_trace_wgs = 0;
   long long* d_clk = nullptr;
   double* d_scratch = nullptr;
+  double* d_scratch2 = nullptr;
+  size_t scratch2_bytes = 0;
+  bool fold_armed = false, fold_events = false;
+  bool fold_busy[2] = {false, false};
+  int fold_sel = 0;
+  hssk_rt::event_t ev_fold{}, ev_fold_done[2] = {};
+  long long dgemm_groups[12] = {0, 0, 0, 0, 0, 0, 0, 0, 0, 0, 0, 0};
   struct hssk_uploader* uploader = nullptr;
   int* d_sweep_flags = nullptr;
   int* h_sweep_err = nullptr;
@@ -130,7 +137,30 @@
       d_scratch = (double*)hssk_rt::dev_malloc(bytes);
       scratch_bytes = bytes;
     }
+    fold_guard(0);
     return d_scratch;
+  }
+  void fold_guard(int r) {
+    if (!fold_busy[r] || on_side) return;
+    hssk_rt::stream_wait_event(stream, ev_fold_done[r]);
+    fold_busy[r] = false;
+  }
+  double* scratch2(size_t bytes) {
+    if (bytes > scratch2_bytes) {
+      sync_all();
+      hssk_rt::dev_free(d_scratch2);
+      d_scratch2 = (double*)hssk_rt::dev_malloc(bytes);
+      scratch2_bytes = bytes;
+    }
+    fold_guard(1);
+    return d_scratch2;
+  }
+  void make_side() {
+    if (side_made) return;
+    side = hssk_rt::stream_create();
+    ev_fork = hssk_rt::event_create();
+    ev_join = hssk_rt::event_create();
+    side_made = true;
   }
 };
 
diff --git a/strumpack_amd/hssk.py b/strumpack_amd/hssk.py
--- a/strumpack_amd/hssk.py
+++ b/strumpack_amd/hssk.py
@@ -160,6 +160,7 @@
     "hssk_cluster_median", "hssk_pchol_id_vbatched", "hssk_pchol_id_max_m", "hssk_pchol_id_rank_cap", "hssk_sum_partials", "hssk_gram_vbatched", "hssk_gram_gen_vbatched", "hssk_gram_gen_supported",
     "hssk_sgemm_sketch", "hssk_narrow_f32", "hssk_gather_elems_f32",
     "hssk_kernel_predict_f32", "hssk_kernel_predict_splits",
+    "hssk_last_dgemm_groups", "hssk_dgemm_fold_next", "hssk_dgemm_fold_join",
 ]
 
 
@@ -230,6 +231,9 @@
         L.hssk_last_dgemm_ms.argtypes = [C.c_void_p]
         L.hssk_last_dgemm_trace.restype = C.c_longlong
         L.hssk_last_dgemm_trace.argtypes = [C.c_void_p, C.c_void_p, C.c_longlong]
+        L.hssk_last_dgemm_groups.argtypes = [C.c_void_p, C.c_void_p]
+        L.hssk_dgemm_fold_next.argtypes = [C.c_void_p]
+        L.hssk_dgemm_fold_join.argtypes = [C.c_void_p]
         L.hssk_last_dgemm_flops.restype = C.c_double
         L.hssk_last_dgemm_flops.argtypes = [C.c_void_p]
         L.hssk_fill_toeplitz.argtypes = [C.c_void_p, C.c_void_p, C.c_int, C.c_longlong, C.c_char]
```

Result: no change. 69290 (-0.3%).
